# nmoehrle/mvs-texturing

Hardware: AMD Instinct MI355X
Metric: faces/sec through view-selection (data-cost + MRF) (higher is better)
Workload: dtype f32

## Files before the change

include/mvs_viewsel_blocks.h:

```cpp
#ifndef MVS_VIEWSEL_BLOCKS_H
#define MVS_VIEWSEL_BLOCKS_H
#include "mvs_viewsel.h"
#ifdef __cplusplus
extern "C" {
#endif

mvs_status mvs_ctx_dc_get_max(mvs_ctx* ctx, float* dst_device);
mvs_status mvs_ctx_dc_set_max(mvs_ctx* ctx, const float* src_device);
mvs_status mvs_ctx_dc_get_histogram(mvs_ctx* ctx, uint32_t* dst_device);
mvs_status mvs_ctx_dc_set_histogram(mvs_ctx* ctx, const uint32_t* src_device);
mvs_status mvs_ctx_costs_export(mvs_ctx* ctx, uint32_t* counts_device, uint16_t* view_id_device, float* cost_device);

enum { MVS_MRF_MSG = 0, MVS_MRF_LAB = 1, MVS_MRF_GAIN = 2, MVS_MRF_BEST_LAB = 3,
       MVS_MRF_MSG_LAB = 4 };
mvs_status mvs_ctx_mrf_setup(mvs_ctx* ctx, const uint32_t* adj_ptr, const uint32_t* adj, int adj_on_device,
                             const mvs_mrf_params* params);
mvs_status mvs_ctx_mrf_sweep_phase(mvs_ctx* ctx, uint32_t phase, uint32_t node_begin, uint32_t node_end);
mvs_status mvs_ctx_mrf_setup_marked(mvs_ctx* ctx, const uint32_t* adj_ptr, const uint32_t* adj, int adj_on_device,
                                    const mvs_mrf_params* params, const uint8_t* marks_device);
mvs_status mvs_ctx_mrf_sweep_phase_part(mvs_ctx* ctx, uint32_t phase, uint32_t node_begin, uint32_t node_end, int part);
mvs_status mvs_ctx_mrf_sweep(mvs_ctx* ctx, uint32_t node_begin, uint32_t node_end);
mvs_status mvs_ctx_mrf_layout(mvs_ctx* ctx, uint32_t* in_off_host, uint64_t n_edges);
mvs_status mvs_ctx_mrf_gather(mvs_ctx* ctx, int which, const uint32_t* idx_device, uint64_t n, void* dst_device);
mvs_status mvs_ctx_mrf_scatter(mvs_ctx* ctx, int which, const uint32_t* idx_device, uint64_t n, const void* src_device);
mvs_status mvs_ctx_mrf_energy(mvs_ctx* ctx, int which_sel, uint32_t node_begin, uint32_t node_end, uint64_t* dst_device);
mvs_status mvs_ctx_mrf_keep_best(mvs_ctx* ctx);
mvs_status mvs_ctx_mrf_step(mvs_ctx* ctx, const uint64_t* energy_device);
mvs_status mvs_ctx_mrf_poll(mvs_ctx* ctx, uint32_t step, mvs_mrf_progress* out);
mvs_status mvs_ctx_mrf_icm_gain(mvs_ctx* ctx, uint32_t node_begin, uint32_t node_end);
mvs_status mvs_ctx_mrf_icm_apply(mvs_ctx* ctx, uint32_t node_begin, uint32_t node_end, uint32_t* moved_device);
mvs_status mvs_ctx_mrf_labels(mvs_ctx* ctx, uint32_t node_begin, uint32_t node_end, uint32_t* labels_device,
                              uint32_t* unseen_out);

#ifdef __cplusplus
}
#endif
#endif
```

mvs-texturing_amd/csrc/api.hip:

```cpp
#include "ctx.h"

#include <atomic>
#include <cmath>
#include <cstdio>
#include <cstdlib>
#include <cstring>
#include <chrono>
#include <mutex>
#include <string>
#include <thread>
#include <vector>

namespace mvs {
void dc_phase1(mvs_ctx* ctx, const mvs_settings* st);
void dc_phase2(mvs_ctx* ctx);
void dc_phase3(mvs_ctx* ctx, mvs_dc_stats* stats);
void undistort_image(mvs_ctx* ctx, const uint8_t* d_src, uint8_t* d_dst, int w, int h, double flen, double d0, double d1);
void dc_prune_labels(mvs_ctx* ctx, uint32_t kmax);
void dc_postprocess(mvs_ctx* ctx, uint32_t nf, uint32_t n_views, const uint32_t* h_ptr, const uint16_t* h_view_rev, const float* h_q_rev, const float* h_col_rev, const mvs_settings* st);
void mrf_setup(mvs_ctx* ctx, const mvs_mrf_params* params);
void mrf_sweep(mvs_ctx* ctx, uint32_t nb0, uint32_t ne0);
void mrf_energy(mvs_ctx* ctx, bool best, uint32_t nb0, uint32_t ne0, bool reduce = true);
void mrf_keep_best(mvs_ctx* ctx);
void mrf_exact_costs(mvs_ctx* ctx, uint32_t nb0, uint32_t ne0);
// ... 192 lines not shown
            if (!ev[k]) MVS_HIP(hipEventCreateWithFlags(&ev[k], hipEventDisableTiming));
        }
    }
    void release() {
        std::lock_guard<std::mutex> lock(m);
        for (unsigned k = 0; k < SLOTS; ++k) { if (ev[k]) (void)hipEventDestroy(ev[k]); if (buf[k]) (void)hipHostFree(buf[k]); ev[k] = nullptr; buf[k] = nullptr; used[k] = false; }
    }
};
constexpr int RING_DEVICES = 16;
UploadRing g_ring[RING_DEVICES];
unsigned upload_threads() {
    if (const char* e = getenv("MVS_UPLOAD_THREADS")) return (unsigned)std::max(1, std::min(atoi(e), (int)UploadRing::MAX_THREADS));
    return std::max(1u, std::min(UploadRing::MAX_THREADS, std::thread::hardware_concurrency() / 2));
}
void upload_through_ring(mvs_ctx* ctx, const std::vector<UploadPiece>& pieces) {
    if (ctx->device < 0 || ctx->device >= RING_DEVICES) throw StatusError(MVS_ERR_UNSUPPORTED, "upload ring: device index out of range");
    UploadRing& R = g_ring[ctx->device];
    std::lock_guard<std::mutex> lock(R.m);
    struct Chunk { const uint8_t* src; uint8_t* dst; size_t n; };
    std::vector<Chunk> chunks;
    for (const UploadPiece& p : pieces) for (size_t o = 0; o < p.bytes; o += UploadRing::SLOT) chunks.push_back(Chunk{p.src + o, p.dst + o, std::min(UploadRing::SLOT, p.bytes - o)});
    const unsigned T = (unsigned)std::max<size_t>(1, std::min<size_t>(upload_threads(), chunks.size()));
    R.ensure(2 * T);
    hipStream_t s = ctx->stream; const int device = ctx->device;
    struct Drain { hipStream_t s; UploadRing& R; ~Drain() { (void)hipStreamSynchronize(s); for (bool& u : R.used) u = false; } } drain{s, R};
    std::mutex em; std::string error; std::atomic<bool> failed{false};
    auto work = [&](unsigned t) {
        try {
            MVS_HIP(hipSetDevice(device));
            unsigned turn = 0;
            for (size_t c = t; c < chunks.size() && !failed.load(std::memory_order_relaxed); c += T, turn ^= 1u) {
                const unsigned k = 2 * t + turn;
                if (R.used[k]) MVS_HIP(hipEventSynchronize(R.ev[k]));
                memcpy(R.buf[k], chunks[c].src, chunks[c].n);
                MVS_HIP(hipMemcpyAsync(chunks[c].dst, R.buf[k], chunks[c].n, hipMemcpyHostToDevice, s));
                MVS_HIP(hipEventRecord(R.ev[k], s));
                R.used[k] = true;
            }
        } catch (const std::exception& e) { failed.store(true); std::lock_guard<std::mutex> l(em); if (error.empty()) error = e.what(); }
    };
    struct Joiner { std::vector<std::thread> th; ~Joiner() { for (auto& x : th) if (x.joinable()) x.join(); } } pool;
    pool.th.reserve(T);
    std::vector<unsigned> mine{0u};
    for (unsigned t = 1; t < T; ++t) {
        try { pool.th.emplace_back(work, t); } catch (const std::system_error&) { mine.push_back(t); }
    }
    for (unsigned t : mine) work(t);
    for (auto& x : pool.th) x.join();
    if (failed.load()) throw HipError("image upload: " + error);
}
}

extern "C" {

const char* mvs_last_error(void) { return g_last_error.c_str(); }

const char* mvs_status_string(mvs_status s) {
    switch (s) {
        case MVS_OK: return "ok";
        case MVS_ERR_INVALID: return "invalid argument";
        case MVS_ERR_TOO_MANY_FACES: return "Exeeded maximal number of faces";
        case MVS_ERR_TOO_MANY_VIEWS: return "Exeeded maximal number of views";
        case MVS_ERR_LABELING: return "Incorrect labeling";
        case MVS_ERR_HIP: return "HIP error";
        case MVS_ERR_STATE: return "invalid call order";
        case MVS_ERR_UNSUPPORTED: return "unsupported";
    }
    return "?";
}

void mvs_mrf_default_params(mvs_mrf_params* p) {
    p->max_sweeps = 200; p->min_sweeps = 20; p->window = 5; p->min_improvement = 0.005f;
    p->damping = 0.2f; p->rho = 0.8f; p->icm_iters = 50; p->region_rounds = 0;
}
void mvs_default_settings(mvs_settings* s) {
    s->data_term = MVS_DATA_TERM_GMI; s->outlier_removal = MVS_OUTLIER_NONE; s->geometric_visibility_test = 1;
}

mvs_status mvs_ctx_create(int device, mvs_ctx** out) {
    if (!out) return fail(MVS_ERR_INVALID, "out is null");
    *out = nullptr;
    MVS_API_BEGIN
    int n = 0;
    if (hipGetDeviceCount(&n) != hipSuccess || n <= 0) throw HipError("no HIP device available (this library has no CPU fallback)");
    if (device < 0 || device >= n) throw StatusError(MVS_ERR_INVALID, "bad device index");
    MVS_HIP(hipSetDevice(device));
    mvs_ctx* c = new mvs_ctx;
    c->device = device;
    MVS_HIP(hipStreamCreateWithFlags(&c->stream, hipStreamNonBlocking));
    c->own_stream = true;
    c->cos_limit = compute_cos_limit();
    if (const char* e = getenv("MVS_INFO_WAVE_AREA")) c->info_wave_area = std::max(0, atoi(e));
    if (const char* e = getenv("MVS_MRF_WIDE")) c->mrf_wide = atoi(e) != 0;
    if (const char* e = getenv("MVS_BVH_UPPER_MIN_FACES")) c->bvh_upper_min_faces = (uint32_t)std::max(0ll, atoll(e));
    c->counters.ensure(64);
    *out = c;
    MVS_API_END
}

void mvs_ctx_destroy(mvs_ctx* ctx) {
    if (!ctx) return;
    (void)hipSetDevice(ctx->device);
    (void)hipStreamSynchronize(ctx->stream);
    for (auto* b : ctx->own_rgb) delete b;
    if (ctx->sweep_exec) (void)hipGraphExecDestroy(ctx->sweep_exec);
    if (ctx->cap_stream) (void)hipStreamDestroy(ctx->cap_stream);
    if (ctx->aux_stream) { (void)hipStreamSynchronize(ctx->aux_stream); (void)hipStreamDestroy(ctx->aux_stream); }
    if (ctx->ev_fork) (void)hipEventDestroy(ctx->ev_fork);
    if (ctx->ev_join) (void)hipEventDestroy(ctx->ev_join);
    if (ctx->h_kd_flags) (void)hipHostFree(ctx->h_kd_flags);
    if (ctx->h_icm) (void)hipHostFree(ctx->h_icm);
    if (ctx->h_rb) (void)hipHostFree(ctx->h_rb);
    if (ctx->h_seq) (void)hipHostFree(ctx->h_seq);
    if (ctx->h_ring) (void)hipHostFree(ctx->h_ring);
    if (ctx->own_stream && ctx->stream) (void)hipStreamDestroy(ctx->stream);
    delete ctx;
}

mvs_status mvs_ctx_set_stream(mvs_ctx* ctx, void* hip_stream) {
    if (!ctx) return fail(MVS_ERR_INVALID, "ctx is null");
    MVS_API_BEGIN
    MVS_HIP(hipStreamSynchronize(ctx->stream));
    if (ctx->own_stream && ctx->stream) MVS_HIP(hipStreamDestroy(ctx->stream));
    ctx->stream = (hipStream_t)hip_stream; ctx->own_stream = false;
    MVS_API_END
}

mvs_status mvs_ctx_synchronize(mvs_ctx* ctx) {
    if (!ctx) return fail(MVS_ERR_INVALID, "ctx is null");
    MVS_API_BEGIN
    MVS_HIP(hipStreamSynchronize(ctx->stream));
    MVS_API_END
}

mvs_status mvs_set_option(mvs_ctx* ctx, const char* name, int64_t value) {
    if (!ctx || !name) return fail(MVS_ERR_INVALID, "null argument");
    const std::string n(name);
    if (n == "count_rays") ctx->count_rays = value != 0;
    else if (n == "stats") ctx->stats = value != 0;
    else if (n == "verbose") ctx->verbose = value != 0;
    else if (n == "info_wave_area") ctx->info_wave_area = (int)std::max<int64_t>(0, std::min<int64_t>(value, 1 << 30));
    else if (n == "info_wave_area_words") ctx->info_wave_area_words = (int)std::max<int64_t>(1, std::min<int64_t>(value, 1 << 30));
    else if (n == "info_words") ctx->info_words = value != 0;
    else if (n == "info_cert_shift") ctx->info_cert_shift = (int)std::max<int64_t>(0, std::min<int64_t>(value, 40));
    else if (n == "max_labels") { if (value < 0 || value > 65535) return fail(MVS_ERR_INVALID, "max_labels: 0 (off) .. 65535"); ctx->max_labels = (int)value; }
    else if (n == "profile") ctx->profile = value != 0;
    else if (n == "prep_fused") ctx->prep_fused = value != 0;
    else if (n == "ray_xcd") ctx->ray_xcd = (int)value;
    else if (n == "mrf_xcd") ctx->mrf_xcd = (int)value;
    else if (n == "mrf_lag") ctx->mrf_lag = (int)value;
    else if (n == "shard_peer_push") ctx->shard_peer_push = value != 0;
    else if (n == "mrf_force_generic") ctx->mrf_force_generic = value != 0;
    else if (n == "mrf_wide") ctx->mrf_wide = value != 0;
    else if (n == "mrf_graph") ctx->mrf_graph = value != 0;
    else if (n == "mrf_late_old") ctx->mrf_late_old = (int)value;
    else if (n == "mrf_damp_period") ctx->mrf_damp_period = (int)std::max<int64_t>(0, std::min<int64_t>(value, 64));
    else if (n == "mrf_run_pad") ctx->mrf_run_pad = (value == 16) ? 16 : 4;
    else if (n == "mrf_blocks_per_cu") ctx->mrf_blocks_per_cu = std::max(0, (int)value);
    else if (n == "bvh_caller_order") ctx->bvh_caller_order = value != 0;
    else if (n == "dc_overlap_prep") ctx->dc_overlap_prep = value != 0;
    else if (n == "bvh_upper_min_faces") { ctx->kd_disabled = false; ctx->bvh_upper_min_faces = (uint32_t)std::max<int64_t>(0, std::min<int64_t>(value, 0xFFFFFFFFll)); ctx->order_pinned = false; }
    else if (n == "bvh_window") { ctx->kd_disabled = false; ctx->bvh_window = (uint32_t)std::max<int64_t>(0, std::min<int64_t>(value, 0x40000000)); ctx->order_pinned = false; }
    else if (n == "face_order") { ctx->face_order = value != 0 ? 1 : 0; ctx->order_pinned = false; }
    else return fail(MVS_ERR_INVALID, "unknown option " + n);
    return MVS_OK;
}

mvs_status mvs_ctx_get_profile(mvs_ctx* ctx, char* buf, size_t buf_size) {
    if (!ctx || !buf || buf_size < 3) return fail(MVS_ERR_INVALID, "null argument");
    MVS_API_BEGIN
    MVS_HIP(hipStreamSynchronize(ctx->stream));
    std::vector<std::string> names; std::vector<double> ms; std::vector<int> cnt;
    for (auto& sp : ctx->prof_spans) {
        float t = 0.0f;
        MVS_HIP(hipEventElapsedTime(&t, sp.a, sp.b));
        size_t k = 0;
        for (; k < names.size(); ++k) if (names[k] == sp.name) break;
        if (k == names.size()) { names.push_back(sp.name); ms.push_back(0.0); cnt.push_back(0); }
        ms[k] += t; cnt[k] += 1;
        if (sp.owns_a) ctx->prof_pool.push_back(sp.a);
        ctx->prof_pool.push_back(sp.b);
    }
    ctx->prof_spans.clear();
    std::string out = "{";
    for (size_t k = 0; k < names.size(); ++k) {
        char tmp[160];
        snprintf(tmp, sizeof(tmp), "%s\"%s\": [%.6f, %d]", k ? ", " : "", names[k].c_str(), ms[k], cnt[k]);
        out += tmp;
    }
    out += "}";
    if (out.size() + 1 > buf_size) throw StatusError(MVS_ERR_INVALID, "profile buffer too small");
    memcpy(buf, out.c_str(), out.size() + 1);
    MVS_API_END
}

mvs_status mvs_scene_set_mesh(mvs_ctx* ctx, const mvs_mesh* mesh, int on_device) {
    if (!ctx || !mesh || !mesh->verts || !mesh->faces || !mesh->face_normals) return fail(MVS_ERR_INVALID, "null argument");
    MVS_API_BEGIN
    MVS_HIP(hipSetDevice(ctx->device));
    const size_t NV = mesh->n_verts, F = mesh->n_faces;
    if (on_device) {
        ctx->d_verts = mesh->verts; ctx->d_faces = mesh->faces; ctx->d_normals = mesh->face_normals;
    } else {
        ctx->own_verts.ensure(3 * NV + 4); ctx->own_faces.ensure(3 * F + 4); ctx->own_normals.ensure(3 * F + 4);
        MVS_HIP(hipMemcpyAsync(ctx->own_verts.p, mesh->verts, 3 * NV * sizeof(float), hipMemcpyHostToDevice, ctx->stream));
        MVS_HIP(hipMemcpyAsync(ctx->own_faces.p, mesh->faces, 3 * F * sizeof(uint32_t), hipMemcpyHostToDevice, ctx->stream));
        MVS_HIP(hipMemcpyAsync(ctx->own_normals.p, mesh->face_normals, 3 * F * sizeof(float), hipMemcpyHostToDevice, ctx->stream));
        MVS_HIP(hipStreamSynchronize(ctx->stream));
        ctx->d_verts = ctx->own_verts.p; ctx->d_faces = ctx->own_faces.p; ctx->d_normals = ctx->own_normals.p;
    }
    ctx->n_verts = mesh->n_verts; ctx->n_faces = mesh->n_faces;
    ctx->face_begin = 0; ctx->face_end = mesh->n_faces;
    ctx->have_costs = false; ctx->dc_phase = 0;
    ctx->order_pinned = false; ctx->iv = nullptr; ctx->kd_disabled = false; ctx->kd_pending = 0;
    MVS_API_END
}

static mvs_status set_views_impl(mvs_ctx* ctx, const mvs_view* views, uint32_t n_views, int rgb_on_device, const mvs_image_source* src);
mvs_status mvs_scene_set_views(mvs_ctx* ctx, const mvs_view* views, uint32_t n_views, int rgb_on_device) { return set_views_impl(ctx, views, n_views, rgb_on_device, nullptr); }
mvs_status mvs_scene_set_views_from(mvs_ctx* ctx, const mvs_view* views, uint32_t n_views, const mvs_image_source* src) {
    if (!src || !src->acquire || !src->release) return fail(MVS_ERR_INVALID, "null argument");
    return set_views_impl(ctx, views, n_views, 0, src);
}
static mvs_status set_views_impl(mvs_ctx* ctx, const mvs_view* views, uint32_t n_views, int rgb_on_device, const mvs_image_source* src) {
    if (!ctx || (!views && n_views)) return fail(MVS_ERR_INVALID, "null argument");
    MVS_API_BEGIN
    MVS_HIP(hipSetDevice(ctx->device));
    if (rgb_on_device) { for (auto* b : ctx->own_rgb) delete b; ctx->own_rgb.clear(); }
    else { while (ctx->own_rgb.size() > n_views) { delete ctx->own_rgb.back(); ctx->own_rgb.pop_back(); } }
    ctx->h_views.assign(n_views, ViewParams{});
    struct Pinned {
        hipStream_t s; std::vector<void*> ptrs;
        ~Pinned() { if (ptrs.empty()) return; (void)hipStreamSynchronize(s); for (void* p : ptrs) (void)hipHostUnregister(p); }
    } pinned{ctx->stream, {}};
    UploadRoute route = rgb_on_device ? UploadRoute::Pageable : upload_route();
    if (src && route == UploadRoute::Register) route = UploadRoute::Ring;
    std::vector<UploadPiece> pieces;
    struct Held {
        const mvs_image_source* src; std::vector<uint32_t> views;
        void release_all() { for (uint32_t j : views) src->release(src->user, j); views.clear(); }
        ~Held() { if (src) release_all(); }
    } held{src, {}};
    const uint32_t in_flight = src ? std::max<uint32_t>(1u, src->max_in_flight ? src->max_in_flight : 4u) : 0u;
    auto flush_batch = [&]() {
        if (!pieces.empty()) upload_through_ring(ctx, pieces);
        pieces.clear();
        MVS_HIP(hipStreamSynchronize(ctx->stream));
        held.release_all();
    };
    for (uint32_t j = 0; j < n_views; ++j) {
        mvs_view v = views[j];
        if (src) {
            if (v.width < 2 || v.height < 2) throw StatusError(MVS_ERR_INVALID, "view " + std::to_string(j) + ": bad image");
            v.rgb = src->acquire(src->user, j);
            if (!v.rgb) throw StatusError(MVS_ERR_INVALID, "view " + std::to_string(j) + ": the image source has no image");
            held.views.push_back(j);
        }
        if (v.width < 2 || v.height < 2 || !v.rgb) throw StatusError(MVS_ERR_INVALID, "view " + std::to_string(j) + ": bad image");
        ViewParams& p = ctx->h_views[j];
        memcpy(p.pos, v.pos, sizeof(p.pos)); memcpy(p.viewdir, v.viewdir, sizeof(p.viewdir));
        memcpy(p.K, v.K, sizeof(p.K)); memcpy(p.w2c, v.w2c, sizeof(p.w2c));
        p.width = v.width; p.height = v.height;
        if (rgb_on_device) p.rgb = v.rgb;
        else {
            if (ctx->own_rgb.size() <= j) ctx->own_rgb.push_back(new DBuf<uint8_t>());
            auto* b = ctx->own_rgb[j];
            const size_t bytes = (size_t)v.width * v.height * 3;
            b->ensure(bytes + 16);
            p.rgb = b->p;
            if (route == UploadRoute::Ring && bytes >= (1u << 18)) { pieces.push_back(UploadPiece{v.rgb, b->p, bytes}); if (src && held.views.size() >= in_flight) flush_batch(); continue; }
            if (route == UploadRoute::Register && bytes >= (1u << 20) && hipHostRegister(const_cast<uint8_t*>(v.rgb), bytes, hipHostRegisterDefault) == hipSuccess) pinned.ptrs.push_back(const_cast<uint8_t*>(v.rgb));
            else (void)hipGetLastError();
            MVS_HIP(hipMemcpyAsync(b->p, v.rgb, bytes, hipMemcpyHostToDevice, ctx->stream));
            if (src && held.views.size() >= in_flight) flush_batch();
        }
    }
    if (src) flush_batch();
    if (!pieces.empty()) upload_through_ring(ctx, pieces);
    MVS_HIP(hipStreamSynchronize(ctx->stream));
    ctx->n_views = n_views;
    ctx->have_costs = false; ctx->dc_phase = 0;
    MVS_API_END
}

mvs_status mvs_scene_set_face_range(mvs_ctx* ctx, uint32_t begin, uint32_t end) {
    if (!ctx) return fail(MVS_ERR_INVALID, "ctx is null");
    if (begin > end || end > ctx->n_faces) return fail(MVS_ERR_INVALID, "bad face range");
    ctx->face_begin = begin; ctx->face_end = end;
    ctx->have_costs = false; ctx->dc_phase = 0;
    return MVS_OK;
}

mvs_status mvs_ctx_dc_phase1(mvs_ctx* ctx, const mvs_settings* settings) {
    if (!ctx || !settings) return fail(MVS_ERR_INVALID, "null argument");
    MVS_API_BEGIN
    MVS_HIP(hipSetDevice(ctx->device));
    dc_phase1(ctx, settings);
    MVS_API_END
}
mvs_status mvs_ctx_dc_phase2(mvs_ctx* ctx) {
    if (!ctx) return fail(MVS_ERR_INVALID, "ctx is null");
    MVS_API_BEGIN
    MVS_HIP(hipSetDevice(ctx->device));
    dc_phase2(ctx);
    MVS_API_END
}
// ... 515 lines not shown
```

mvs-texturing_amd/csrc/ctx.h:

```cpp
#pragma once
#include <hip/hip_runtime.h>
#include <stdint.h>
#include <string.h>
#include <algorithm>
#include <stdexcept>
#include <string>
#include <vector>

#include "../../include/mvs_viewsel.h"
#include "dmath.h"

namespace mvs {

struct HipError : std::runtime_error {
    explicit HipError(const std::string& m) : std::runtime_error(m) {}
};
struct StatusError : std::runtime_error {
    mvs_status st;
    StatusError(mvs_status s, const std::string& m) : std::runtime_error(m), st(s) {}
};

#define MVS_HIP(expr)                                                                          \
    do {                                                                                       \
        hipError_t _e = (expr);                                                                \
// ... 39 lines not shown
    HBuf() = default;
    HBuf(const HBuf&) = delete;
    HBuf& operator=(const HBuf&) = delete;
};

struct alignas(128) Node4 {
    float b[4][6];
    uint32_t nchild;
    uint32_t pad_[7];
    __host__ __device__ float lo(int a, int c) const { return b[c][a]; }
    __host__ __device__ float hi(int a, int c) const { return b[c][3 + a]; }
};
static_assert(sizeof(Node4) == 128, "Node4 must be one 128-byte line");

struct BvhDev {
    const Node4* nodes;
    const float4* tris;
    uint32_t level_off[16];
    uint32_t level_cnt[16];
    int32_t top;
    uint32_t n_leaves;
};

struct ProfSpan { std::string name; hipEvent_t a, b; bool owns_a; };

struct MrfEdge {
    uint32_t in_off;
    uint32_t out_off;
    uint32_t kj;
};

struct alignas(16) NodeDesc {
    uint32_t rec;
    uint32_t id;
    uint32_t in_off[3];
    uint32_t out_off[3];
    uint32_t kk;
    uint32_t nbr[3];
};
static_assert(sizeof(NodeDesc) == 48, "NodeDesc must be 48 bytes");

}

struct mvs_ctx {
    int device = 0;
    hipStream_t stream = nullptr;
    bool own_stream = false;
    bool verbose = false;
    bool profile = false;
    std::vector<mvs::ProfSpan> prof_spans; std::vector<hipEvent_t> prof_pool;
    bool prep_fused = true;
    bool stats = false;
    bool count_rays = false;
    bool dc_overlap_prep = true;
    uint32_t* h_kd_flags = nullptr; int kd_pending = 0; bool kd_disabled = false;
    uint32_t* h_rb = nullptr; uint32_t* d_rb = nullptr; uint32_t rb_seq = 0;
    hipStream_t aux_stream = nullptr; hipEvent_t ev_fork = nullptr, ev_join = nullptr;
    uint32_t bvh_upper_min_faces = 1000000;
    uint32_t bvh_window = 262144;
    mvs::DBuf<float> kd_c[2][3]; mvs::DBuf<uint32_t> kd_id[2], kd_hist, kd_cursor, kd_tie, kd_pivot, kd_box;
    bool bvh_caller_order = false;
    int ray_xcd = 1;
    int info_wave_area = 32;
    int info_wave_area_words = 384;
    bool info_words = true;
    int info_cert_shift = 0;
    uint32_t dc_stats_deferred = 0;
    int max_labels = 0;
    float cos_limit = 0.0f;

    uint32_t n_verts = 0, n_faces = 0, n_views = 0;
    uint32_t face_begin = 0, face_end = 0;
    const float* d_verts = nullptr; const uint32_t* d_faces = nullptr; const float* d_normals = nullptr;
    mvs::DBuf<float> own_verts, own_normals; mvs::DBuf<uint32_t> own_faces;
    std::vector<mvs::ViewParams> h_views;
    mvs::DBuf<mvs::ViewParams> d_views;
    std::vector<mvs::DBuf<uint8_t>*> own_rgb;
    mvs::DBuf<uint8_t> gmi_all;
    mvs::DBuf<uint8_t> lum_all;
    mvs::DBuf<uint32_t> mask_all;
    mvs::DBuf<uint32_t> mask_zero, mask_tmp;
    mvs::DBuf<uint32_t> msum_all;
    std::vector<size_t> gmi_off, mask_off, msum_off;
    mvs::DBuf<size_t> view_off;
    bool mesh_dirty = true, views_dirty = true;

    int face_order = 1;
    mvs::DBuf<float> i_verts, i_normals; mvs::DBuf<uint32_t> i_faces, f_perm, f_pos, f_tmp;
    const float* iv = nullptr; const uint32_t* ifc = nullptr; const float* inr = nullptr;
    bool mesh_ordered = false;
    bool order_pinned = false;
    const uint32_t* t_perm = nullptr; const uint32_t* t_pos = nullptr;
    mvs::DBuf<uint32_t> u_ptr, u_cnt; mvs::DBuf<uint16_t> u_view; mvs::DBuf<float> u_cost, u_q;
    bool u_valid = false, u_q_valid = false;
    mvs::DBuf<unsigned long long> fp_acc;
    mvs::HBuf<uint32_t> stage_ptr; mvs::HBuf<uint16_t> stage_view[2]; mvs::HBuf<float> stage_cost[2];

    mvs::DBuf<mvs::Node4> bvh_nodes; mvs::DBuf<float4> bvh_tris;
    mvs::DBuf<uint32_t> sort_k, sort_k2, sort_v, sort_v2; mvs::DBuf<char> sort_tmp;
    mvs::DBuf<float> lvl_box_a, lvl_box_b; mvs::DBuf<float> scene_box;
    mvs::BvhDev bvh{};
    mvs::DBuf<uint32_t> vf_ptr, vf_cursor, vf;
    mvs::DBuf<uint32_t> vperm, vpos;
    const uint32_t* tri_order = nullptr;

    mvs::DBuf<unsigned long long> pass_bits, need_bits, occl_bits, surv_bits;
    mvs::DBuf<uint32_t> pass_base;
    mvs::DBuf<uint32_t> pass_face;
    mvs::DBuf<unsigned long long> defer_bits; mvs::DBuf<uint32_t> defer_base; mvs::DBuf<uint2> defer_list; mvs::DBuf<uint32_t> rewalk_list;
    mvs::DBuf<float> pq;
    mvs::DBuf<float> pcol;
    mvs::DBuf<uint32_t> face_cnt, scan_tmp;
    mvs::DBuf<unsigned long long> counters;
    mvs::DBuf<float> max_q; mvs::DBuf<uint32_t> hist; mvs::DBuf<float> pctl;
    mvs::DBuf<uint32_t> pre_ptr; mvs::DBuf<uint16_t> pre_view; mvs::DBuf<float> pre_q; mvs::DBuf<float> pre_col;
    mvs::DBuf<uint8_t> pre_inl;
    mvs::DBuf<uint32_t> csr_ptr; mvs::DBuf<uint16_t> csr_view; mvs::DBuf<float> csr_cost; mvs::DBuf<float> csr_q;
    uint32_t csr_faces = 0, csr_views = 0; uint64_t csr_nnz = 0;
    const uint32_t* r_ptr = nullptr; const uint16_t* r_view = nullptr; const float* r_cost = nullptr;
    bool csr_q_valid = false;
    bool have_costs = false;
    mvs_settings dc_settings{}; mvs_dc_stats dc_stats{}; int dc_phase = 0;

    mvs::DBuf<unsigned long long> g_keys, g_keys2; mvs::DBuf<uint32_t> g_vals, g_vals2, g_pos, g_cnt, g_adj_ptr, g_adj, g_faces; mvs::DBuf<float> g_normals;
    uint64_t g_adj_entries = 0; bool have_adj = false;

    mvs::DBuf<uint32_t> p_label_ptr, p_comp_ptr, p_comp_faces, p_parent, p_root, p_state, p_flag, p_pos, p_roots, p_roots2, p_rlab, p_rlab2, p_adj_ptr, p_adj, p_labels;

    mvs::DBuf<uint32_t> rg_parent, rg_root, rg_size, rg_bestl, rg_lose, rg_flag, rg_pos, rg_cstart, rg_have, rg_cfirst, rg_name;
    mvs::DBuf<unsigned long long> rg_gain, rg_cur, rg_key, rg_key2, rg_ck, rg_sum; mvs::DBuf<long long> rg_cgain; mvs::DBuf<uint2> rg_cut;

    mvs::DBuf<uint32_t> m_adj_ptr, m_adj, a_stage_ptr, a_stage; const uint32_t* r_adj_ptr = nullptr; const uint32_t* r_adj = nullptr;
    uint32_t r_adj_edges = 0; bool r_adj_edges_known = false;
    mvs::DBuf<mvs::NodeDesc> m_desc; mvs::DBuf<uint8_t> m_ident; mvs::DBuf<uint32_t> m_rec; uint64_t m_rec_words = 0; bool m_fast = false; int mrf_blocks_per_cu = 0 , mrf_xcd = 1, mrf_late_old = 1, mrf_run_pad = 4;
    mvs::DBuf<mvs::MrfEdge> m_edge; mvs::DBuf<uint32_t> m_size, m_rev ; mvs::DBuf<uint16_t> m_map;
    mvs::DBuf<uint8_t> m_msg_a;
    mvs::DBuf<uint32_t> m_sel, m_sel2, m_cand; mvs::DBuf<float> m_gain;
    mvs::DBuf<uint32_t> m_lab; mvs::DBuf<float> m_cost;
    uint32_t m_stride = 0;
    bool exact_valid = false; uint32_t exact_nb = 0, exact_ne = 0;
    uint32_t* b_sel = nullptr; uint32_t* b_lab = nullptr; float* b_cost = nullptr; bool best_resolved = false;
    mvs::DBuf<unsigned long long> m_energy; mvs::DBuf<uint32_t> m_moved; mvs::DBuf<uint32_t> m_alist; bool icm_dirty_valid = false;
    uint32_t m_n_adj = 0;
    uint32_t m_energy_blocks = 0;
    bool m_energy_from_sweep = false;
    uint64_t m_total = 0; uint32_t m_kmax = 0, m_degmax = 0;
    mvs::DBuf<uint32_t> m_colour, m_perm, m_tmp_a, m_tmp_b, m_tmp_c, m_sub; mvs::DBuf<uint8_t> m_cls; uint32_t m_colours = 0, m_n_fast = 0; std::vector<uint32_t> m_sub_begin;
    const uint32_t* m_colour_in = nullptr;
    const uint8_t* m_bnd = nullptr;
    int mrf_damp_period = 4;
    int mrf_force_generic = 0;
    int mrf_wide = 1;
    bool m_wide_layout = false;
    uint32_t m_range_nb = 0, m_range_ne = 0; std::vector<uint32_t> m_range_q;
    uint32_t m_sweep_no = 0;
    mvs_mrf_params m_params{};
    static constexpr uint32_t RING = 16;
    static constexpr uint32_t ICM_RING = 8;
    uint32_t* h_icm = nullptr; uint32_t* d_icm = nullptr; uint32_t icm_seq = 0;
    mvs::DBuf<mvs_mrf_progress> m_state; mvs::DBuf<unsigned long long> m_hist; mvs::DBuf<uint32_t> m_ctl;
    int mrf_graph = 1; hipStream_t cap_stream = nullptr; hipGraphExec_t sweep_exec = nullptr; uint32_t graph_launches = 0, graph_updates = 0, graph_instantiations = 0;
    mvs_mrf_progress* h_ring = nullptr; mvs_mrf_progress* d_ring = nullptr ; uint32_t steps_issued = 0; int mrf_lag = 1;
    int shard_peer_push = 1;
    uint32_t* h_seq = nullptr; uint32_t* d_seq = nullptr; uint32_t seq_base = 0;
};

namespace mvs {
struct Prof {
    mvs_ctx* c; size_t idx; bool on;
    Prof(mvs_ctx* ctx, const char* name) : c(ctx), idx(0), on(ctx->profile) {
        if (!on) return;
        auto get = [&]() { hipEvent_t e; if (!c->prof_pool.empty()) { e = c->prof_pool.back(); c->prof_pool.pop_back(); } else { MVS_HIP(hipEventCreate(&e)); } return e; };
        ProfSpan sp{name, get(), get(), true};
        MVS_HIP(hipEventRecord(sp.a, c->stream));
        idx = c->prof_spans.size(); c->prof_spans.push_back(sp);
    }
    void end() { if (on) { MVS_HIP(hipEventRecord(c->prof_spans[idx].b, c->stream)); on = false; } }
    ~Prof() { if (on) (void)hipEventRecord(c->prof_spans[idx].b, c->stream); }
};
struct ProfChain {
    mvs_ctx* c; hipEvent_t prev; bool on;
    static hipEvent_t get(mvs_ctx* c) { hipEvent_t e; if (!c->prof_pool.empty()) { e = c->prof_pool.back(); c->prof_pool.pop_back(); } else { MVS_HIP(hipEventCreate(&e)); } return e; }
    explicit ProfChain(mvs_ctx* ctx) : c(ctx), prev(nullptr), on(ctx->profile) {}
    void begin() { if (on && !prev) { prev = get(c); MVS_HIP(hipEventRecord(prev, c->stream)); first = true; } }
    void mark(const char* name) {
        if (!on) return;
        begin();
        hipEvent_t e = get(c);
        MVS_HIP(hipEventRecord(e, c->stream));
        c->prof_spans.push_back(ProfSpan{name, prev, e, first});
        first = false; prev = e;
    }
    bool first = false;
};
struct RoctxRange { explicit RoctxRange(const char* name); ~RoctxRange(); bool on; };
int default_device();
enum { MRF_PART_ALL = 0, MRF_PART_BOUNDARY = 1, MRF_PART_INTERIOR = 2 };
void ensure_report_ring(mvs_ctx* ctx);
void report_u32(mvs_ctx* ctx, const uint32_t* d_src, uint32_t* d_dst, uint32_t seq_slot, uint32_t seq);
void wait_report(mvs_ctx* ctx, uint32_t seq_slot, uint32_t seq);
void read_words(mvs_ctx* ctx, const void* d_src, void* out, uint32_t n_words);
void read_block(mvs_ctx* ctx, const void* d_src, void* out, size_t bytes);
void exclusive_scan_u32(mvs_ctx* ctx, const uint32_t* in, uint32_t* out, size_t n, uint32_t* d_total);
uint64_t sum_u32(mvs_ctx* ctx, const uint32_t* in, size_t n);
}
```

mvs-texturing_amd/csrc/k_mrf.hip:

```cpp
#include "ctx.h"
#include <rocprim/rocprim.hpp>
#include <atomic>

namespace mvs {

namespace {

constexpr uint16_t MAP_NONE = 0xFFFF;
constexpr uint32_t MSG_BASE = MVS_MRF_MSG_BASE;

typedef uint8_t msg_t;
struct MsgQ { float scale, step; };
__device__ __forceinline__ MsgQ msg_q(float lam) { return MsgQ{255.0f / lam, lam / 255.0f}; }
template <class T> __device__ __forceinline__ T ld_off(const void* base, uint32_t byte_off) { return *reinterpret_cast<const T*>(reinterpret_cast<const char*>(base) + byte_off); }
template <class T> __device__ __forceinline__ void st_off(void* base, uint32_t byte_off, T v) { *reinterpret_cast<T*>(reinterpret_cast<char*>(base) + byte_off) = v; }
__device__ __forceinline__ float min_raw(float a, float b) { float r; asm("v_min_f32 %0, %1, %2" : "=v"(r) : "v"(a), "v"(b)); return r; }
template <bool DAMP>
__device__ __forceinline__ uint32_t msg_pack_s(float raw_s, float alpha, float old_code, uint32_t byte, uint32_t word) {
    return __builtin_amdgcn_cvt_pk_u8_f32(DAMP ? __builtin_fmaf(old_code, alpha, raw_s) : raw_s, byte, word);
}
template <bool DAMP>
__device__ __forceinline__ uint32_t msg_pack(float raw, float oms, float alpha, float old_code, uint32_t byte, uint32_t word) {
    const float v = DAMP ? __builtin_fmaf(old_code, alpha, raw * oms) : raw * oms;
    return __builtin_amdgcn_cvt_pk_u8_f32(v, byte, word);
// ... 167 lines not shown
        for (int t = 0; t < 4; ++t) { oj[t] = orig ? orig[j[t]] : j[t]; cj[t] = __hip_atomic_load(colour + j[t], __ATOMIC_RELAXED, __HIP_MEMORY_SCOPE_AGENT); }
#pragma unroll
        for (int t = 0; t < 4; ++t) {
            if (j[t] == i || !mrf_key_less(oj[t], oi)) continue;
            if (cj[t] == NO_COLOUR) ready = false; else used |= 1ull << cj[t];
        }
    }
    if (ready) {
        if (used == ~0ull) { pending[1] = 1u; used = 0ull; }
        __hip_atomic_store(colour + i, (uint32_t)__builtin_ctzll(~used), __ATOMIC_RELAXED, __HIP_MEMORY_SCOPE_AGENT);
    } else *pending = 1u;
}
constexpr uint32_t N_SUB = 320;
constexpr uint32_t SUB_GENERIC = 256;
constexpr uint32_t N_KEY = 2 * N_SUB;
__global__ void mrf_sortkey_kernel(const uint32_t* __restrict__ colour, const uint8_t* __restrict__ cls, const uint8_t* __restrict__ bnd, uint32_t F, uint32_t* __restrict__ key) {
    const uint32_t i = blockIdx.x * blockDim.x + threadIdx.x;
    if (i < F) { const uint32_t c = colour[i], k = cls[i]; key[i] = 2u * ((k == CLS_GENERIC) ? SUB_GENERIC + c : 4u * c + k) + ((bnd && bnd[i]) ? 0u : 1u); }
}
__global__ void mrf_sub_begin_kernel(const uint32_t* __restrict__ sorted, uint32_t F, uint32_t* __restrict__ sub_begin) {
    const uint32_t c = blockIdx.x * blockDim.x + threadIdx.x;
    if (c > N_KEY) return;
    uint32_t lo = 0, hi = F;
    while (lo < hi) { const uint32_t mid = (lo + hi) >> 1; if (sorted[mid] < c) lo = mid + 1; else hi = mid; }
    sub_begin[c] = lo;
}
__global__ void mrf_sub_range_kernel(const uint32_t* __restrict__ perm, const uint32_t* __restrict__ sub_begin,
                                     uint32_t nb, uint32_t ne, uint32_t* __restrict__ out) {
    const uint32_t c = blockIdx.x * blockDim.x + threadIdx.x;
    if (c >= N_KEY) return;
    const uint32_t cb = sub_begin[c], ce = sub_begin[c + 1];
    uint32_t lo = cb, hi = ce;
    while (lo < hi) { const uint32_t mid = (lo + hi) >> 1; if (perm[mid] < nb) lo = mid + 1; else hi = mid; }
    out[2 * c] = lo;
    hi = ce;
    while (lo < hi) { const uint32_t mid = (lo + hi) >> 1; if (perm[mid] < ne) lo = mid + 1; else hi = mid; }
    out[2 * c + 1] = lo;
}
constexpr int MAX_LAYOUT_COLOURS = 8;
__global__ void mrf_nodesize_kernel(const uint32_t* __restrict__ perm, const uint32_t* __restrict__ colour, const uint32_t* __restrict__ adj_ptr,
                                    const uint32_t* __restrict__ adj, const uint32_t* __restrict__ size, const uint32_t* __restrict__ rev, uint32_t F, uint32_t n_col,
                                    uint32_t* __restrict__ nsz) {
    const uint32_t q = blockIdx.x * blockDim.x + threadIdx.x;
    if (q > F) return;
    uint32_t acc[MAX_LAYOUT_COLOURS];
#pragma unroll
    for (int b = 0; b < MAX_LAYOUT_COLOURS; ++b) acc[b] = 0;
    if (q < F) {
        const uint32_t j = perm[q];
        const uint32_t ra = adj_ptr[j], rz = adj_ptr[j + 1];
        for (uint32_t rb = ra; rb < rz; rb += 4) {
            uint32_t i[4], e[4], b[4], sz[4];
#pragma unroll
            for (int t = 0; t < 4; ++t) { const bool on = rb + t < rz; i[t] = on ? adj[rb + t] : j; e[t] = on ? rev[rb + t] : 0xFFFFFFFFu; }
#pragma unroll
            for (int t = 0; t < 4; ++t) { b[t] = (n_col > 1) ? colour[i[t]] : 0u; sz[t] = (e[t] != 0xFFFFFFFFu) ? size[e[t]] : 0u; }
#pragma unroll
            for (int t = 0; t < 4; ++t)
#pragma unroll
                for (int c = 0; c < MAX_LAYOUT_COLOURS; ++c) acc[c] += ((uint32_t)c == b[t]) ? sz[t] : 0u;
        }
    }
#pragma unroll
    for (int b = 0; b < MAX_LAYOUT_COLOURS; ++b) if ((uint32_t)b < n_col) nsz[(size_t)b * (F + 1) + q] = acc[b];
}
__global__ void mrf_inoff_kernel(const uint32_t* __restrict__ perm, const uint32_t* __restrict__ colour, const uint32_t* __restrict__ adj_ptr,
                                 const uint32_t* __restrict__ adj, const uint32_t* __restrict__ size, const uint32_t* __restrict__ rev, const uint32_t* __restrict__ noff,
                                 uint32_t F, uint32_t n_col, uint32_t* __restrict__ in_off) {
    const uint32_t q = blockIdx.x * blockDim.x + threadIdx.x;
    if (q >= F) return;
    const uint32_t j = perm[q];
    uint32_t off[MAX_LAYOUT_COLOURS];
#pragma unroll
    for (int b = 0; b < MAX_LAYOUT_COLOURS; ++b) off[b] = ((uint32_t)b < n_col) ? noff[(size_t)b * (F + 1) + q] : 0u;
    const uint32_t ra = adj_ptr[j], rz = adj_ptr[j + 1];
    for (uint32_t rb = ra; rb < rz; rb += 4) {
        uint32_t i[4], e[4], b[4], sz[4];
#pragma unroll
        for (int t = 0; t < 4; ++t) { const bool on = rb + t < rz; i[t] = on ? adj[rb + t] : j; e[t] = on ? rev[rb + t] : 0xFFFFFFFFu; }
#pragma unroll
        for (int t = 0; t < 4; ++t) { b[t] = (n_col > 1) ? colour[i[t]] : 0u; sz[t] = (e[t] != 0xFFFFFFFFu) ? size[e[t]] : 0u; }
#pragma unroll
        for (int t = 0; t < 4; ++t) {
            if (e[t] == 0xFFFFFFFFu) continue;
            uint32_t o = 0;
#pragma unroll
            for (int c = 0; c < MAX_LAYOUT_COLOURS; ++c) { if ((uint32_t)c == b[t]) { o = off[c]; off[c] += sz[t]; } }
            in_off[e[t]] = o;
        }
    }
}

__global__ void mrf_edge_kernel(const uint32_t* __restrict__ col_ptr, const uint32_t* __restrict__ adj_ptr, const uint32_t* __restrict__ adj,
                                uint32_t F, const uint32_t* __restrict__ in_off, const uint32_t* __restrict__ size, const uint32_t* __restrict__ rev, MrfEdge* __restrict__ edge) {
    const uint32_t i = blockIdx.x * blockDim.x + threadIdx.x;
    if (i >= F) return;
    const uint32_t e0 = adj_ptr[i], e1 = adj_ptr[i + 1];
    for (uint32_t eb = e0; eb < e1; eb += 4) {
        uint32_t j[4], r[4], io[4], sz[4], oo[4], kj[4];
#pragma unroll
        for (int t = 0; t < 4; ++t) { const bool on = eb + t < e1; j[t] = on ? adj[eb + t] : i; r[t] = on ? rev[eb + t] : 0xFFFFFFFFu; io[t] = on ? in_off[eb + t] : 0u; sz[t] = on ? size[eb + t] : 0u; }
#pragma unroll
        for (int t = 0; t < 4; ++t) { oo[t] = (r[t] != 0xFFFFFFFFu) ? in_off[r[t]] : 0u; kj[t] = col_ptr[j[t] + 1] - col_ptr[j[t]]; }
#pragma unroll
        for (int t = 0; t < 4; ++t) {
            if (eb + t >= e1) continue;
            const bool has = r[t] != 0xFFFFFFFFu;
            MrfEdge m;
            m.in_off = MSG_BASE + io[t];
            m.out_off = has ? MSG_BASE + oo[t] : 0u;
            m.kj = (sz[t] > 0 && has) ? kj[t] : 0u;
            edge[eb + t] = m;
        }
    }
}

constexpr uint32_t MAP_TILE = 256;
__global__ void __launch_bounds__(256) mrf_map_kernel(const uint32_t* __restrict__ col_ptr, const uint16_t* __restrict__ view_id, const uint32_t* __restrict__ adj_ptr,
                               const uint32_t* __restrict__ adj, uint32_t F, const MrfEdge* __restrict__ edge, const uint8_t* __restrict__ cls, uint16_t* __restrict__ map) {
    __shared__ uint16_t s_l[16][MAP_TILE];
    const uint32_t i = (blockIdx.x * blockDim.x + threadIdx.x) >> 4;
    const uint32_t gl = threadIdx.x & 15;
    if (i >= F) return;
    uint16_t* tile = s_l[threadIdx.x >> 4];
    const uint32_t p0 = col_ptr[i], K = col_ptr[i + 1] - p0;
    for (uint32_t e = adj_ptr[i]; e < adj_ptr[i + 1]; ++e) {
        const MrfEdge m = edge[e];
        if (m.kj == 0 || cls[adj[e]] != CLS_GENERIC) continue;
        const uint32_t q0 = col_ptr[adj[e]];
        const bool in_lds = m.kj <= MAP_TILE;
        if (in_lds) for (uint32_t t = gl; t < m.kj; t += 16) tile[t] = view_id[q0 + t];
        for (uint32_t t = gl; t < K; t += 16) {
            const uint16_t key = view_id[p0 + t];
            uint32_t lo = 0, hi = m.kj;
            if (in_lds) { while (lo < hi) { const uint32_t mid = (lo + hi) >> 1; if (tile[mid] < key) lo = mid + 1; else hi = mid; } }
            else { while (lo < hi) { const uint32_t mid = (lo + hi) >> 1; if (view_id[q0 + mid] < key) lo = mid + 1; else hi = mid; } }
            const uint16_t found = (lo < m.kj) ? (in_lds ? tile[lo] : view_id[q0 + lo]) : (uint16_t)0;
            map[m.in_off + t] = (lo < m.kj && found == key) ? (uint16_t)lo : MAP_NONE;
        }
    }
}

constexpr uint32_t REC_BASE = 256;
constexpr float COST_SCALE = 65535.0f;
__device__ __forceinline__ uint32_t cost_code(float c) { return (uint32_t)(c * COST_SCALE + 0.5f); }
__device__ __forceinline__ float cost_value(uint32_t code) { return (float)code * (1.0f / 65535.0f); }
__device__ __forceinline__ uint32_t label_position(const uint16_t* __restrict__ view_id, uint32_t p0, uint32_t K, uint32_t l) {
    uint32_t lo = 0, hi = K;
    const uint32_t key = l - 1u;
    while (lo < hi) { const uint32_t mid = (lo + hi) >> 1; if ((uint32_t)view_id[p0 + mid] < key) lo = mid + 1; else hi = mid; }
    return lo < K ? lo : K - 1u;
}

__global__ void __launch_bounds__(256) mrf_ident_kernel(const uint32_t* __restrict__ col_ptr, const uint16_t* __restrict__ view_id, const uint32_t* __restrict__ adj_ptr,
                                                        const uint32_t* __restrict__ adj, uint32_t F, const MrfEdge* __restrict__ edge, const uint8_t* __restrict__ cls,
                                                        uint8_t* __restrict__ ident) {
    const uint32_t i = (blockIdx.x * blockDim.x + threadIdx.x) >> 4;
    const uint32_t gl = threadIdx.x & 15;
    if (i >= F || cls[i] == CLS_GENERIC) return;
    const uint32_t p0 = col_ptr[i], K = col_ptr[i + 1] - p0;
    const uint32_t e0 = adj_ptr[i], e1 = adj_ptr[i + 1];
    for (uint32_t e = e0; e < e1; e += 3) {
        uint32_t kj[3], q0[3];
#pragma unroll
        for (int k = 0; k < 3; ++k) {
            const bool on = e + k < e1;
            kj[k] = on ? edge[e + k].kj : 0u;
            q0[k] = col_ptr[on ? adj[e + k] : i];
        }
        uint32_t same = 0;
#pragma unroll
        for (int k = 0; k < 3; ++k) same |= (kj[k] != 0u && kj[k] == K) ? (1u << k) : 0u;
        if (same) {
            for (uint32_t t = gl; t < K; t += 16) {
                const uint32_t v = view_id[p0 + t];
#pragma unroll
                for (int k = 0; k < 3; ++k)
                    if ((same >> k) & 1u) { if (view_id[q0[k] + t] != v) same &= ~(1u << k); }
            }
            for (int o = 8; o > 0; o >>= 1) same &= __shfl_xor(same, o, 16);
        }
        if (gl < 3 && e + gl < e1 && kj[gl] != 0u) ident[e + gl] = (uint8_t)((same >> gl) & 1u);
    }
}
__global__ void mrf_recsize_kernel(const uint32_t* __restrict__ col_ptr, const uint32_t* __restrict__ adj_ptr, const MrfEdge* __restrict__ edge,
                                   const uint8_t* __restrict__ ident, const uint8_t* __restrict__ cls, const uint32_t* __restrict__ perm, uint32_t F, uint32_t wide,
                                   uint32_t* __restrict__ rsz, uint32_t* __restrict__ qpos) {
    const uint32_t q = blockIdx.x * blockDim.x + threadIdx.x;
    if (q > F) return;
    uint32_t w = 0;
    if (q < F) {
        const uint32_t i = perm[q], K = col_ptr[i + 1] - col_ptr[i];
        qpos[i] = q;
        if (K && cls[i] != CLS_GENERIC) {
            w = (K + 3u) & ~3u;
            const bool w8 = wide != 0u && cls[i] == 1u;
            const uint32_t e0 = adj_ptr[i], e1 = adj_ptr[i + 1];
            for (uint32_t eb = e0; eb < e1; eb += 4) {
                uint32_t kj[4], id[4];
#pragma unroll
                for (int t = 0; t < 4; ++t) { const bool on = eb + t < e1; kj[t] = on ? edge[eb + t].kj : 0u; id[t] = on ? ident[eb + t] : 1u; }
#pragma unroll
                for (int t = 0; t < 4; ++t) if (kj[t] && !id[t]) w += w8 ? 2u * ((kj[t] + 7u) >> 3) : (kj[t] + 3u) >> 2;
            }
            w = (w + 3u) & ~3u;
        }
    }
    rsz[q] = w;
}
__global__ void __launch_bounds__(256) mrf_record_kernel(const uint32_t* __restrict__ col_ptr, const uint16_t* __restrict__ view_id, const float* __restrict__ cost,
                                                         const uint32_t* __restrict__ adj_ptr, const uint32_t* __restrict__ adj, const MrfEdge* __restrict__ edge,
                                                         const uint8_t* __restrict__ ident, const uint8_t* __restrict__ cls, const uint32_t* __restrict__ qpos, const uint32_t* __restrict__ roff,
                                                         uint32_t F, uint32_t wide, uint32_t* __restrict__ rec) {
    __shared__ uint16_t s_l[16][256];
    const uint32_t i = (blockIdx.x * blockDim.x + threadIdx.x) >> 4;
    const uint32_t gl = threadIdx.x & 15;
    if (i >= F) return;
    const uint32_t p0 = col_ptr[i], K = col_ptr[i + 1] - p0;
    const uint32_t ci = cls[i];
    if (K == 0 || ci == CLS_GENERIC) return;
    const bool w8 = wide != 0u && ci == 1u;
    const uint32_t rs = w8 ? 8u : 8u << ci, none_byte = w8 ? 64u : (ci < 3u ? 4u * rs : 0xFFu);
    const uint32_t lmask = w8 ? 7u : 3u, lshift = w8 ? 3u : 2u;
    const uint32_t q = qpos[i];
    uint16_t* tile = s_l[threadIdx.x >> 4];
    uint32_t* out = rec + REC_BASE + roff[q];
    const uint32_t K4 = (K + 3u) & ~3u;
    const uint32_t e0 = adj_ptr[i], deg = adj_ptr[i + 1] - e0;
    uint32_t kj3[3], q03[3];
    {
        uint32_t kj[3], idn[3], nb[3];
#pragma unroll
        for (uint32_t d = 0; d < 3; ++d) { const bool on = d < deg; kj[d] = on ? edge[e0 + d].kj : 0u; idn[d] = on ? (uint32_t)ident[e0 + d] : 1u; nb[d] = on ? adj[e0 + d] : i; }
#pragma unroll
        for (uint32_t d = 0; d < 3; ++d) { kj3[d] = (kj[d] != 0u && idn[d] == 0u) ? kj[d] : 0u; q03[d] = col_ptr[nb[d]]; }
    }
    for (uint32_t t = gl; t < K4; t += 16) {
        uint32_t w = 0u;
        if (t < K) { const uint32_t v = view_id[p0 + t]; tile[t] = (uint16_t)v; w = (cost_code(cost[p0 + t]) << 16) | v; }
        out[t] = w;
    }
    uint32_t pos = K4;
#pragma unroll
    for (uint32_t d = 0; d < 3; ++d) {
        const uint32_t kj = kj3[d];
        if (kj == 0) continue;
        const uint32_t q0 = q03[d], nw = w8 ? 2u * ((kj + 7u) >> 3) : (kj + 3u) >> 2;
        for (uint32_t wI = gl; wI < nw; wI += 16) {
            uint32_t key[4], lo[4] = {0u, 0u, 0u, 0u};
#pragma unroll
            for (uint32_t r = 0; r < 4; ++r) { const uint32_t t2 = 4u * wI + r; key[r] = (t2 < kj) ? (uint32_t)view_id[q0 + t2] : 0xFFFFFFFFu; }
            for (uint32_t n = K; n > 1u;) {
                const uint32_t half = n >> 1;
#pragma unroll
                for (uint32_t r = 0; r < 4; ++r) lo[r] += ((uint32_t)tile[lo[r] + half - 1u] < key[r]) ? half : 0u;
                n -= half;
            }
            uint32_t word = 0u;
#pragma unroll
            for (uint32_t r = 0; r < 4; ++r) {
                uint32_t at = lo[r] + (((uint32_t)tile[lo[r]] < key[r]) ? 1u : 0u);
                const uint32_t byte = (at < K && (uint32_t)tile[at < K ? at : 0u] == key[r]) ? (at & lmask) * rs + (at >> lshift) : none_byte;
                word |= byte << (8 * r);
            }
            out[pos + wI] = word;
        }
        pos += nw;
    }
    for (uint32_t t = pos + gl; t < ((pos + 3u) & ~3u); t += 16) out[t] = 0u;
}
__global__ void mrf_desc_kernel(const uint32_t* __restrict__ col_ptr, const uint32_t* __restrict__ adj_ptr, const uint32_t* __restrict__ adj,
                                const MrfEdge* __restrict__ edge, const uint8_t* __restrict__ ident, const uint32_t* __restrict__ perm,
                                const uint32_t* __restrict__ colour, const uint32_t* __restrict__ roff, uint32_t n_fast, NodeDesc* __restrict__ desc) {
    const uint32_t q = blockIdx.x * blockDim.x + threadIdx.x;
    if (q >= n_fast) return;
    const uint32_t i = perm[q];
    NodeDesc nd;
    const uint32_t k = col_ptr[i + 1] - col_ptr[i];
    nd.rec = k ? REC_BASE + roff[q] : 0u; nd.id = i; nd.kk = k;
    const uint32_t e0 = adj_ptr[i], deg = adj_ptr[i + 1] - e0, ci = colour[i];
    for (int d = 0; d < 3; ++d) {
        MrfEdge m; m.in_off = 0; m.out_off = 0; m.kj = 0;
        uint32_t flag_ident = 0, flag_low = 0, nb = i;
        if ((uint32_t)d < deg) { nb = adj[e0 + d]; flag_low = (colour[nb] < ci) ? 1u : 0u; }
        if ((uint32_t)d < deg && k > 0) {
            m = edge[e0 + d];
            if (m.kj && ident[e0 + d]) flag_ident = 1u;
            if (m.kj == 0) { m.in_off = 0; m.out_off = 0; }
        }
        nd.in_off[d] = m.in_off | flag_low; nd.out_off[d] = m.out_off | flag_ident; nd.kk |= m.kj << (8 + 8 * d); nd.nbr[d] = nb;
    }
    desc[q] = nd;
}

template <int G, bool DAMP, bool XCD, bool LATE_OLD>
__global__ void __launch_bounds__(256) mrf_sweep4_kernel(const NodeDesc* __restrict__ desc, const uint32_t* __restrict__ rec, msg_t* msg,
                                                         const mvs_mrf_progress* __restrict__ st, uint32_t* lab2, uint32_t buf_stride,
                                                         uint32_t node_begin , uint32_t node_end, float rho, float alpha,
                                                         unsigned long long* __restrict__ partial) {
    const msg_t* mo = msg; msg_t* mn = msg;
    constexpr int NPB = 256 / G;
    constexpr int TS = G == 8 ? 40 : G == 16 ? 80 : 4 * G + 4;
    __shared__ float s_c[NPB * TS];
    __shared__ unsigned long long s_e[8];
    const int grp = threadIdx.x / G, gl = threadIdx.x % G;
    float* __restrict__ tile = s_c + grp * TS;
    if (st->stopped) return;
    if (gl == 0) tile[4 * G] = INFINITY;
    __syncthreads();
    const uint32_t wofs = st->w * buf_stride;
    uint32_t* lab = lab2 + wofs;
    const float lam = 1.0f / rho;
    const MsgQ mq = msg_q(lam);
    const float kappa = rho * mq.step, nstep = -mq.step, oms = (1.0f - alpha) * mq.scale, lam_s = lam * oms;
    constexpr float HUGE_COST = 1e30f;
    const uint32_t stride = gridDim.x * NPB;
    uint32_t vb = blockIdx.x;
    if (XCD && (gridDim.x & 7u) == 0u) vb = (blockIdx.x & 7u) * (gridDim.x >> 3) + (blockIdx.x >> 3);
    uint32_t i = node_begin + vb * NPB + grp;
    const uint32_t last = node_end - 1;
    const uint32_t n_iter = (node_end - node_begin + stride - 1) / stride;
    const uint32_t t0 = 4u * gl;
    const uint32_t ident_word = 0x03020100u * (uint32_t)G + 0x01010101u * (uint32_t)gl;
    struct Raw { uint4 lw; uint32_t in[3], map[3], nl[3], old[3]; };
    const uint32_t t0b = 4u * t0, glb = 4u * (uint32_t)gl;
    auto issue = [&](const NodeDesc& d, Raw& r) {
        const uint32_t K = d.kk & 0xFFu, recb = 4u * d.rec;
        r.lw = ld_off<uint4>(rec, recb + t0b);
        uint32_t mposb = recb + 4u * ((K + 3u) & ~3u) + glb;
#pragma unroll
        for (int e = 0; e < 3; ++e) {
            r.in[e] = ld_off<uint32_t>(mo, (d.in_off[e] & ~3u) + t0);
            r.map[e] = ld_off<uint32_t>(rec, mposb);
            if (!(d.out_off[e] & 1u)) mposb += (((d.kk >> (8 + 8 * e)) & 0xFFu) + 3u) & ~3u;
            r.nl[e] = ld_off<uint32_t>(lab, 4u * d.nbr[e]);
            if (DAMP) r.old[e] = ld_off<uint32_t>(mo, (d.out_off[e] & ~3u) + t0); else r.old[e] = d.out_off[e];
        }
    };
    NodeDesc cur = ld_off<NodeDesc>(desc, (uint32_t)sizeof(NodeDesc) * min(i, last));
    Raw rw; issue(cur, rw);
    NodeDesc nxt = ld_off<NodeDesc>(desc, (uint32_t)sizeof(NodeDesc) * min(i + stride, last));
    uint32_t acc_e = 0u, acc_c = 0u;
#pragma unroll 2
    for (uint32_t it = 0; it < n_iter; ++it, i += stride) {
        const bool node_ok = i < node_end;
        Raw rn; issue(nxt, rn);
        const NodeDesc nn = ld_off<NodeDesc>(desc, (uint32_t)sizeof(NodeDesc) * min(i + 2u * stride, last));
        const uint32_t K = node_ok ? (cur.kk & 0xFFu) : 0u;
        bool ok[4];
#pragma unroll
        for (int r = 0; r < 4; ++r) ok[r] = t0 + r < K;
        uint32_t kj3[3], o_out[3]; bool ident[3], low[3];
#pragma unroll
        for (int d = 0; d < 3; ++d) {
            kj3[d] = node_ok ? ((cur.kk >> (8 + 8 * d)) & 0xFFu) : 0u;
            ident[d] = (cur.out_off[d] & 1u) != 0u; low[d] = (cur.in_off[d] & 1u) != 0u && kj3[d] != 0u;
            o_out[d] = cur.out_off[d] & ~3u;
        }
        const uint32_t lw[4] = {rw.lw.x, rw.lw.y, rw.lw.z, rw.lw.w};
        const uint32_t* r_in = rw.in; const uint32_t* r_map = rw.map; const uint32_t* nl = rw.nl; const uint32_t* r_old = rw.old;
        float cf[3][4], b[4];
#pragma unroll
        for (int r = 0; r < 4; ++r) {
#pragma unroll
            for (int d = 0; d < 3; ++d) cf[d][r] = (float)((r_in[d] >> (8 * r)) & 0xFFu);
            const float D = ok[r] ? cost_value(lw[r] >> 16) : HUGE_COST;
            b[r] = __builtin_fmaf(kappa, (cf[0][r] + cf[1][r]) + cf[2][r], D);
        }
        float cv[3][4];
#pragma unroll
        for (int d = 0; d < 3; ++d)
#pragma unroll
            for (int r = 0; r < 4; ++r) cv[d][r] = __builtin_fmaf(nstep, cf[d][r], b[r]) * oms;
        float gm = fminf(fminf(b[0], b[1]), fminf(b[2], b[3]));
        float cm0 = fminf(fminf(cv[0][0], cv[0][1]), fminf(cv[0][2], cv[0][3])), cm1 = fminf(fminf(cv[1][0], cv[1][1]), fminf(cv[1][2], cv[1][3])),
              cm2 = fminf(fminf(cv[2][0], cv[2][1]), fminf(cv[2][2], cv[2][3]));
        group_min_fused4<G>(gm, cm0, cm1, cm2);
        const float cmin3[3] = {cm0, cm1, cm2};
        uint32_t bt = (b[3] == gm) ? t0 + 3u : 0xFFFFFFFFu;
        bt = (b[2] == gm) ? t0 + 2u : bt; bt = (b[1] == gm) ? t0 + 1u : bt; bt = (b[0] == gm) ? t0 : bt;
        bt = group_min_fused<G>(bt);
#pragma unroll
        for (int d = 0; d < 3; ++d) {
#pragma unroll
            for (int r = 0; r < 4; ++r) tile[r * G + gl] = cv[d][r] - cmin3[d];
            const uint32_t mw = ident[d] ? ident_word : r_map[d];
            uint32_t w = 0u;
#pragma unroll
            for (int r = 0; r < 4; ++r) {
                const uint32_t mp = (mw >> (8 * r)) & 0xFFu;
                const uint32_t slot = (G < 64) ? mp : ((mp == 0xFFu) ? (uint32_t)(4 * G) : mp);
                w = msg_pack_s<DAMP>(min_raw(tile[slot], lam_s), alpha, (float)((r_old[d] >> (8 * r)) & 0xFFu), (uint32_t)r, w);
            }
            if (t0 < kj3[d]) st_off<uint32_t>(mn, o_out[d] + t0, w);
        }
        const bool owner = node_ok && ((K > 0u) ? ((bt >> 2) == (uint32_t)gl) : (gl == 0));
        if (owner) {
            const uint32_t r = bt & 3u;
            const uint32_t wsel = (r == 0u) ? lw[0] : (r == 1u) ? lw[1] : (r == 2u) ? lw[2] : lw[3];
            const uint32_t my_lab = (K > 0u) ? (wsel & 0xFFFFu) + 1u : 0u;
            const uint32_t my_code = (K > 0u) ? (wsel >> 16) : 65535u;
            const uint32_t idb = 4u * cur.id;
            st_off<uint32_t>(lab, idb, my_lab);
            acc_e += my_code;
// ... 329 lines not shown
__global__ void __launch_bounds__(256) mrf_icm_apply_kernel(const uint32_t* __restrict__ col_ptr, const uint16_t* __restrict__ view_id, const float* __restrict__ cost,
                                                            const uint32_t* __restrict__ adj_ptr, const uint32_t* __restrict__ adj,
                                                            const float* __restrict__ gain, const uint32_t* __restrict__ cand,
                                                            uint32_t* sel, uint32_t* lab, float* selcost,
                                                            uint32_t node_begin, uint32_t node_end, uint32_t* __restrict__ moved ,
                                                            uint32_t* __restrict__ alist ,
                                                            const uint32_t* __restrict__ orig ) {
    const uint32_t i = node_begin + blockIdx.x * blockDim.x + threadIdx.x;
    bool mv = false;
    if (i < node_end) {
        const float gi = gain[i];
        if (gi > 0.0f) {
            bool win = true;
            for (uint32_t e = adj_ptr[i]; e < adj_ptr[i + 1] && win; ++e) {
                const uint32_t j = adj[e];
                if (lab[j] == 0u) continue;
                const float gj = gain[j];
                if (gj > gi || (gj == gi && (orig ? orig[j] < orig[i] : j < i))) win = false;
            }
            if (win) mv = true;
        }
    }
    if (mv) {
        const uint32_t p0 = col_ptr[i], t = cand[i];
        sel[i] = t; lab[i] = (uint32_t)view_id[p0 + t] + 1u; selcost[i] = cost[p0 + t];
        if (alist) {
            const uint32_t e0 = adj_ptr[i], e1 = adj_ptr[i + 1];
            uint32_t w = atomicAdd(&moved[1], 1u + (e1 - e0));
            alist[w++] = i;
            for (uint32_t e = e0; e < e1; ++e) alist[w++] = adj[e];
        }
    }
    const unsigned long long b = __ballot(mv);
    if ((threadIdx.x & 63) == 0 && b) atomicAdd(moved, (uint32_t)__popcll(b));
}

__global__ void mrf_argmin_unary_kernel(const uint32_t* __restrict__ col_ptr, const uint16_t* __restrict__ view_id, const float* __restrict__ cost, uint32_t F,
                                        uint32_t* __restrict__ sel, uint32_t* __restrict__ lab, float* __restrict__ selcost) {
    const uint32_t i = blockIdx.x * blockDim.x + threadIdx.x;
    if (i >= F) return;
    const uint32_t p0 = col_ptr[i], K = col_ptr[i + 1] - p0;
    uint32_t bt = 0;
    for (uint32_t t = 1; t < K; ++t) if (cost[p0 + t] < cost[p0 + bt]) bt = t;
    sel[i] = bt;
    lab[i] = K ? (uint32_t)view_id[p0 + bt] + 1u : 0u;
    selcost[i] = K ? cost[p0 + bt] : 1.0f;
}

__global__ void mrf_labels_kernel(const uint32_t* __restrict__ lab, uint32_t node_begin, uint32_t node_end, uint32_t n_views,
                                  uint32_t* __restrict__ labels, uint32_t* __restrict__ bad_unseen ,
                                  const uint32_t* __restrict__ orig ,
                                  const uint32_t* __restrict__ foreign ) {
    const uint32_t i = node_begin + blockIdx.x * blockDim.x + threadIdx.x;
    if (i >= node_end) return;
    if (foreign && i == node_begin && *foreign) atomicAdd(&bad_unseen[0], *foreign);
    const uint32_t label = lab[i];
    if (label > n_views) atomicAdd(&bad_unseen[0], 1u);
    if (label == 0u) atomicAdd(&bad_unseen[1], 1u);
    labels[orig ? orig[i] : i - node_begin] = label;
}


__global__ void __launch_bounds__(1024) mrf_step_kernel(mvs_mrf_progress* __restrict__ st, unsigned long long* __restrict__ hist,
                                const unsigned long long* __restrict__ energy, const unsigned long long* __restrict__ partial, uint32_t n_partial,
                                unsigned long long* __restrict__ energy_out, mvs_mrf_progress* __restrict__ ring, uint32_t* __restrict__ ring_seq, uint32_t ring_slots,
                                uint32_t* __restrict__ ctl, int max_sweeps, int min_sweeps, int window, float min_improvement,
                                const unsigned long long* const* __restrict__ peer_tab = nullptr, uint32_t n_peer = 0, uint32_t peer_off = 0) {
    __shared__ unsigned long long su[16], sc[16];
    unsigned long long e_sum = 0, c_sum = 0;
    if (partial) {
        const ulonglong2* pp = reinterpret_cast<const ulonglong2*>(partial);
#pragma unroll 8
        for (uint32_t b = threadIdx.x; b < n_partial; b += 1024u) { const ulonglong2 v = pp[b]; e_sum += v.x; c_sum += v.y; }
        for (int o = 32; o > 0; o >>= 1) { e_sum += __shfl_xor(e_sum, o, 64); c_sum += __shfl_xor(c_sum, o, 64); }
        if ((threadIdx.x & 63) == 0) { su[threadIdx.x >> 6] = e_sum; sc[threadIdx.x >> 6] = c_sum; }
        __syncthreads();
    }
    if (threadIdx.x != 0 || blockIdx.x != 0) return;
    if (partial) {
        e_sum = 0; c_sum = 0;
        for (int k = 0; k < 16; ++k) { e_sum += su[k]; c_sum += sc[k]; }
        energy_out[0] = e_sum; energy_out[1] = c_sum;
    } else if (peer_tab) {
        e_sum = 0; c_sum = 0;
        for (uint32_t q = 0; q < n_peer; ++q) { e_sum += peer_tab[q][peer_off]; c_sum += peer_tab[q][peer_off + 1u]; }
        energy_out[0] = e_sum; energy_out[1] = c_sum;
    }
    mvs_mrf_progress p = *st;
    if (p.stopped) { p.improved = 0u; }
    else {
        const uint32_t sw = p.sweep + 1u;
        const unsigned long long e0 = (partial || peer_tab) ? e_sum : energy[0];
        const bool imp = e0 < p.best;
        if (imp) { p.best = e0; p.best_w = p.w; p.w ^= 1u; }
        p.sweep = sw; p.improved = imp ? 1u : 0u; p.energy = e0;
        hist[sw] = p.best;
        bool stop = false;
        if ((int)sw >= min_sweeps && (int)sw > window) {
            const unsigned long long prev = hist[sw - (uint32_t)window];
            stop = (double)(prev - p.best) < (double)min_improvement * (double)prev;
        }
        if ((int)sw >= max_sweeps) stop = true;
        if (stop) { p.stopped = 1u; p.stop_sweep = sw; }
    }
    *st = p;
    const uint32_t n = ctl[0] + 1u; ctl[0] = n;
    if (ring) {
        const uint32_t slot = n % ring_slots;
        ring[slot] = p;
        __threadfence_system();
        __hip_atomic_store(ring_seq + slot, ctl[1] + n, __ATOMIC_RELEASE, __HIP_MEMORY_SCOPE_SYSTEM);
    }
}
__global__ void report_u32_kernel(const uint32_t* __restrict__ src, uint32_t* __restrict__ dst, uint32_t* __restrict__ dst_seq, uint32_t seq) {
    *dst = *src;
    __threadfence_system();
    __hip_atomic_store(dst_seq, seq, __ATOMIC_RELEASE, __HIP_MEMORY_SCOPE_SYSTEM);
}
__global__ void report_words_kernel(const uint32_t* __restrict__ src, uint32_t n, uint32_t* __restrict__ dst, uint32_t* __restrict__ dst_seq, uint32_t seq) {
    if (threadIdx.x < n) dst[threadIdx.x] = src[threadIdx.x];
    __threadfence_system();
    __syncthreads();
    if (threadIdx.x == 0) __hip_atomic_store(dst_seq, seq, __ATOMIC_RELEASE, __HIP_MEMORY_SCOPE_SYSTEM);
}
__global__ void mrf_flip_kernel(mvs_mrf_progress* __restrict__ st) { st->best_w = st->w; st->w ^= 1u; }

}

constexpr uint32_t EPART_BLOCKS = 2048;

void mrf_setup(mvs_ctx* ctx, const mvs_mrf_params* params) {
    hipStream_t s = ctx->stream;
    const uint32_t F = ctx->csr_faces;
    ctx->m_params = *params;
    if (!(params->rho > 0.0f && params->rho <= 1.0f) || !(params->damping >= 0.0f && params->damping < 1.0f))
        throw StatusError(MVS_ERR_INVALID, "mrf params: need 0 < rho <= 1, 0 <= damping < 1");
    if (params->window < 1 || params->min_sweeps < 0 || !(params->min_improvement >= 0.0f) || params->icm_iters < 0)
        throw StatusError(MVS_ERR_INVALID, "mrf params: need window >= 1, min_sweeps >= 0, min_improvement >= 0, icm_iters >= 0");
    uint32_t E = ctx->r_adj_edges;
    if (!ctx->r_adj_edges_known) {
        MVS_HIP(hipMemcpyAsync(&E, ctx->r_adj_ptr + F, sizeof(uint32_t), hipMemcpyDeviceToHost, s));
        MVS_HIP(hipStreamSynchronize(s));
    }
    ctx->m_size.ensure((size_t)E + 2); ctx->m_edge.ensure((size_t)E + 1); ctx->m_moved.ensure(8 + 2 * 64);
    ctx->m_n_adj = E;
    uint32_t* maxes = ctx->m_moved.p + 4;
    MVS_HIP(hipMemsetAsync(ctx->m_moved.p, 0, 8 * sizeof(uint32_t), s));
    MVS_HIP(hipMemsetAsync(ctx->m_size.p, 0, ((size_t)E + 2) * sizeof(uint32_t), s));
    const unsigned nb = (F + 255) / 256;
    const uint32_t force_generic = (ctx->csr_nnz < 4 || E == 0 || ctx->mrf_force_generic) ? 1u : 0u;
    ctx->m_cls.ensure((size_t)F + 4);
    ctx->m_rev.ensure((size_t)E + 2);
    if (F) { hipLaunchKernelGGL(mrf_size_kernel, dim3(nb), dim3(256), 0, s, ctx->r_ptr, ctx->r_adj_ptr, ctx->r_adj, F, (uint32_t)(ctx->mrf_run_pad == 16 ? 15 : (ctx->mrf_wide ? 7 : 3)), force_generic, ctx->m_size.p, ctx->m_cls.p, maxes, ctx->m_rev.p); MVS_LAUNCH_CHECK(); }
    ctx->m_colour.ensure((size_t)F + 2); ctx->m_perm.ensure((size_t)F + 2); ctx->m_tmp_a.ensure((size_t)MAX_LAYOUT_COLOURS * ((size_t)F + 1) + 72); ctx->m_tmp_b.ensure((size_t)MAX_LAYOUT_COLOURS * ((size_t)F + 1) + 2); ctx->m_tmp_c.ensure((size_t)F + 2);
    ctx->m_colours = 0; ctx->m_sub_begin.assign(N_KEY + 1, 0); ctx->m_n_fast = 0; ctx->m_range_q.clear(); ctx->m_range_nb = ctx->m_range_ne = 0;
    ctx->m_sweep_no = 0;
    if (F) {
        uint32_t* pending = ctx->m_moved.p + 1;
        hipLaunchKernelGGL(mrf_colour_init_kernel, dim3(nb), dim3(256), 0, s, ctx->m_colour.p, ctx->m_tmp_a.p , F); MVS_LAUNCH_CHECK();
        if (ctx->m_colour_in) MVS_HIP(hipMemcpyAsync(ctx->m_colour.p, ctx->m_colour_in, (size_t)F * sizeof(uint32_t), hipMemcpyDeviceToDevice, s));
        for (int round = 0; !ctx->m_colour_in; ++round) {
            if (round >= 4096) throw StatusError(MVS_ERR_HIP, "graph colouring did not terminate");
            MVS_HIP(hipMemsetAsync(pending, 0, sizeof(uint32_t), s));
            for (int k = 0; k < (round == 0 ? 16 : 4); ++k) { hipLaunchKernelGGL(mrf_colour_round_kernel, dim3(nb), dim3(256), 0, s, ctx->r_adj_ptr, ctx->r_adj, ctx->t_perm, F, ctx->m_colour.p, pending); MVS_LAUNCH_CHECK(); }
            uint32_t hp[2] = {0, 0};
            read_words(ctx, pending, hp, 2);
            if (hp[1]) throw StatusError(MVS_ERR_UNSUPPORTED, "adjacency graph needs more than 64 colours (a node with >= 64 mutually constrained neighbours)");
            if (!hp[0]) break;
        }
        MVS_HIP(hipMemsetAsync(ctx->m_moved.p, 0, 4 * sizeof(uint32_t), s));
        hipLaunchKernelGGL(mrf_sortkey_kernel, dim3(nb), dim3(256), 0, s, ctx->m_colour.p, ctx->m_cls.p, ctx->m_bnd, F, ctx->m_tmp_c.p); MVS_LAUNCH_CHECK();
        size_t tmp_bytes = 0;
        MVS_HIP(rocprim::radix_sort_pairs(nullptr, tmp_bytes, ctx->m_tmp_c.p, ctx->m_tmp_b.p, ctx->m_tmp_a.p, ctx->m_perm.p, F, 0, 10, s));
        ctx->sort_tmp.ensure(tmp_bytes + 16);
        MVS_HIP(rocprim::radix_sort_pairs(ctx->sort_tmp.p, tmp_bytes, ctx->m_tmp_c.p, ctx->m_tmp_b.p, ctx->m_tmp_a.p, ctx->m_perm.p, F, 0, 10, s));
        ctx->m_sub.ensure(3 * (size_t)N_KEY + 8);
        hipLaunchKernelGGL(mrf_sub_begin_kernel, dim3((N_KEY + 256) / 256), dim3(256), 0, s, ctx->m_tmp_b.p, F, ctx->m_sub.p); MVS_LAUNCH_CHECK();
        read_block(ctx, ctx->m_sub.p, ctx->m_sub_begin.data(), (N_KEY + 1) * sizeof(uint32_t));
        const std::vector<uint32_t>& sb = ctx->m_sub_begin;
        uint32_t C = 0;
        for (uint32_t c = 0; c < 64; ++c) if (sb[2 * (4 * c + 4)] > sb[2 * (4 * c)] || sb[2 * (SUB_GENERIC + c + 1)] > sb[2 * (SUB_GENERIC + c)]) C = c + 1;
        ctx->m_colours = C;
        ctx->m_n_fast = sb[2 * SUB_GENERIC];
    }
    DBuf<uint32_t>& in_off = ctx->m_sel2;
    in_off.ensure(std::max<size_t>((size_t)E + 2, (size_t)F + 2));
    MVS_HIP(hipMemsetAsync(in_off.p, 0, ((size_t)E + 2) * sizeof(uint32_t), s));
    uint32_t h[3] = {0, 0, 0};
    if (F) {
        if ((uint64_t)E * 4ull + 4ull * (uint64_t)ctx->csr_nnz >= 0xFFFFFFF0ull) {
            const uint64_t total = sum_u32(ctx, ctx->m_size.p, (size_t)E + 1);
            if ((uint64_t)MSG_BASE + total >= 0xFFFFFFF0ull) throw StatusError(MVS_ERR_UNSUPPORTED, "message array exceeds 2^32 elements (shard the graph: DESIGN.md multi-GPU)");
        }
        const uint32_t n_col = (ctx->m_colours >= 2 && ctx->m_colours <= (uint32_t)MAX_LAYOUT_COLOURS) ? ctx->m_colours : 1u;
        const size_t n_ent = (size_t)n_col * ((size_t)F + 1);
        ctx->m_tmp_a.ensure(n_ent + 72); ctx->m_tmp_b.ensure(n_ent + 2);
        hipLaunchKernelGGL(mrf_nodesize_kernel, dim3((F + 256) / 256), dim3(256), 0, s, ctx->m_perm.p, ctx->m_colour.p, ctx->r_adj_ptr, ctx->r_adj, ctx->m_size.p, ctx->m_rev.p, F, n_col, ctx->m_tmp_a.p); MVS_LAUNCH_CHECK();
        exclusive_scan_u32(ctx, ctx->m_tmp_a.p, ctx->m_tmp_b.p, n_ent, nullptr);
        hipLaunchKernelGGL(mrf_inoff_kernel, dim3(nb), dim3(256), 0, s, ctx->m_perm.p, ctx->m_colour.p, ctx->r_adj_ptr, ctx->r_adj, ctx->m_size.p, ctx->m_rev.p, ctx->m_tmp_b.p, F, n_col, in_off.p); MVS_LAUNCH_CHECK();
        MVS_HIP(hipMemcpyAsync(maxes + 2, ctx->m_tmp_b.p + (n_ent - 1), sizeof(uint32_t), hipMemcpyDeviceToDevice, s));
    } else MVS_HIP(hipMemsetAsync(maxes + 2, 0, sizeof(uint32_t), s));
    { uint32_t hm[3]; read_words(ctx, maxes, hm, 3); h[1] = hm[0]; h[2] = hm[1]; h[0] = hm[2]; }
    ctx->m_total = (uint64_t)MSG_BASE + h[0]; ctx->m_kmax = h[1]; ctx->m_degmax = h[2];
    if (ctx->m_total >= 0xFFFFFFF0ull) throw StatusError(MVS_ERR_UNSUPPORTED, "message array exceeds 2^32 elements");
    if (F) { hipLaunchKernelGGL(mrf_edge_kernel, dim3(nb), dim3(256), 0, s, ctx->r_ptr, ctx->r_adj_ptr, ctx->r_adj, F, in_off.p, ctx->m_size.p, ctx->m_rev.p, ctx->m_edge.p); MVS_LAUNCH_CHECK(); }
    ctx->m_ident.ensure((size_t)E + 1);
    MVS_HIP(hipMemsetAsync(ctx->m_ident.p, 0, (size_t)E + 1, s));
    ctx->m_fast = true;
    ctx->m_wide_layout = ctx->mrf_wide != 0;
    const uint32_t n_fast = ctx->m_n_fast, n_generic = F - n_fast;
    if (n_fast) {
        const size_t rec_cap = (size_t)REC_BASE + ctx->csr_nnz + 8 * (size_t)F + ctx->m_total / 4 + (ctx->mrf_wide ? (size_t)ctx->m_n_adj : 0) + 1024;
        ctx->m_rec.ensure(rec_cap);
        MVS_HIP(hipMemsetAsync(ctx->m_rec.p, 0, REC_BASE * sizeof(uint32_t), s));
        hipLaunchKernelGGL(mrf_ident_kernel, dim3((unsigned)(((size_t)F * 16 + 255) / 256)), dim3(256), 0, s, ctx->r_ptr, ctx->r_view, ctx->r_adj_ptr, ctx->r_adj, F, ctx->m_edge.p, ctx->m_cls.p, ctx->m_ident.p); MVS_LAUNCH_CHECK();
        uint32_t* rsz = ctx->m_tmp_a.p; uint32_t* roff = ctx->m_tmp_b.p;
        hipLaunchKernelGGL(mrf_recsize_kernel, dim3((F + 256) / 256), dim3(256), 0, s, ctx->r_ptr, ctx->r_adj_ptr, ctx->m_edge.p, ctx->m_ident.p, ctx->m_cls.p, ctx->m_perm.p, F, (uint32_t)(ctx->mrf_wide ? 1 : 0), rsz, ctx->m_tmp_c.p); MVS_LAUNCH_CHECK();
        exclusive_scan_u32(ctx, rsz, roff, (size_t)F + 1, nullptr);
        hipLaunchKernelGGL(mrf_record_kernel, dim3((unsigned)(((size_t)F * 16 + 255) / 256)), dim3(256), 0, s, ctx->r_ptr, ctx->r_view, ctx->r_cost, ctx->r_adj_ptr, ctx->r_adj,
                           ctx->m_edge.p, ctx->m_ident.p, ctx->m_cls.p, ctx->m_tmp_c.p , roff, F, (uint32_t)(ctx->mrf_wide ? 1 : 0), ctx->m_rec.p); MVS_LAUNCH_CHECK();
        ctx->m_desc.ensure((size_t)F + 1);
        hipLaunchKernelGGL(mrf_desc_kernel, dim3((n_fast + 255) / 256), dim3(256), 0, s, ctx->r_ptr, ctx->r_adj_ptr, ctx->r_adj, ctx->m_edge.p, ctx->m_ident.p, ctx->m_perm.p, ctx->m_colour.p, roff, n_fast, ctx->m_desc.p); MVS_LAUNCH_CHECK();
    }
    if (n_generic) {
        ctx->m_map.ensure(ctx->m_total + 8);
        hipLaunchKernelGGL(mrf_map_kernel, dim3((unsigned)(((size_t)F * 16 + 255) / 256)), dim3(256), 0, s, ctx->r_ptr, ctx->r_view, ctx->r_adj_ptr, ctx->r_adj, F, ctx->m_edge.p, ctx->m_cls.p, ctx->m_map.p); MVS_LAUNCH_CHECK();
        ctx->pq.ensure(ctx->csr_nnz + 1);
    }
    ctx->m_msg_a.ensure(ctx->m_total + 1024);
    MVS_HIP(hipMemsetAsync(ctx->m_msg_a.p, 0, (ctx->m_total + 1024) * sizeof(msg_t), s));
    const size_t F1 = (size_t)F + 1;
    ctx->m_stride = (uint32_t)F1;
    ctx->m_sel.ensure(2 * F1); ctx->m_lab.ensure(2 * F1); ctx->m_cost.ensure(2 * F1);
    ctx->m_sel2.ensure(F1); ctx->m_cand.ensure(F1); ctx->m_gain.ensure(F1);
    MVS_HIP(hipMemsetAsync(ctx->m_sel.p, 0, 2 * F1 * sizeof(uint32_t), s));
    MVS_HIP(hipMemsetAsync(ctx->m_lab.p, 0, 2 * F1 * sizeof(uint32_t), s));
    MVS_HIP(hipMemsetAsync(ctx->m_cost.p, 0, 2 * F1 * sizeof(float), s));
    mvs_mrf_progress init; memset(&init, 0, sizeof(init)); init.best = ~0ull; init.energy = ~0ull; init.w = 0u; init.best_w = 1u;
    if (F && params->max_sweeps <= 0) {
        hipLaunchKernelGGL(mrf_argmin_unary_kernel, dim3(nb), dim3(256), 0, s, ctx->r_ptr, ctx->r_view, ctx->r_cost, F, ctx->m_sel.p, ctx->m_lab.p, ctx->m_cost.p);
        MVS_LAUNCH_CHECK();
        init.w = 1u; init.best_w = 0u;
    }
    ctx->b_sel = ctx->m_sel.p + init.best_w * F1; ctx->b_lab = ctx->m_lab.p + init.best_w * F1; ctx->b_cost = ctx->m_cost.p + init.best_w * F1;
    ctx->best_resolved = true;
    MVS_HIP(hipMemsetAsync(ctx->m_gain.p, 0, F1 * sizeof(float), s));
    const size_t epart = 4 + 2 * (size_t)EPART_BLOCKS * std::max<size_t>(ctx->m_colours, 1);
    ctx->m_energy.ensure(epart);
    MVS_HIP(hipMemsetAsync(ctx->m_energy.p, 0, epart * sizeof(unsigned long long), s));
    ctx->m_state.ensure(1); ctx->m_hist.ensure((size_t)std::max(params->max_sweeps, 0) + 2);
    ensure_report_ring(ctx);
    ctx->seq_base += ctx->steps_issued;
    ctx->h_ring[mvs_ctx::RING] = init;
    MVS_HIP(hipMemcpyAsync(ctx->m_state.p, &ctx->h_ring[mvs_ctx::RING], sizeof(init), hipMemcpyHostToDevice, s));
    ctx->m_ctl.ensure(4);
    uint32_t* stage = ctx->h_seq + (mvs_ctx::RING + mvs_ctx::ICM_RING);
    stage[0] = 0u; stage[1] = ctx->seq_base;
    MVS_HIP(hipMemcpyAsync(ctx->m_ctl.p, stage, 2 * sizeof(uint32_t), hipMemcpyHostToDevice, s));
    MVS_HIP(hipMemsetAsync(ctx->m_hist.p, 0xFF, sizeof(unsigned long long), s));
    ctx->steps_issued = 0; ctx->icm_dirty_valid = false; ctx->exact_valid = false;
}

void resolve_best(mvs_ctx* ctx) {
    if (ctx->best_resolved) return;
    if (!ctx->m_state.p) throw StatusError(MVS_ERR_STATE, "mrf setup first");
    mvs_mrf_progress p;
    static_assert(sizeof(p) % 4 == 0 && sizeof(p) <= 64, "mvs_mrf_progress travels through read_words");
    read_words(ctx, ctx->m_state.p, &p, (uint32_t)(sizeof(p) / 4));
    const size_t o = (size_t)(p.best_w & 1u) * ctx->m_stride;
    ctx->b_sel = ctx->m_sel.p + o; ctx->b_lab = ctx->m_lab.p + o; ctx->b_cost = ctx->m_cost.p + o;
    ctx->best_resolved = true;
}

void mrf_step(mvs_ctx* ctx, const unsigned long long* energy, const unsigned long long* const* peer_tab, uint32_t n_peer, uint32_t peer_off) {
    hipStream_t s = ctx->stream;
    const mvs_mrf_params& P = ctx->m_params;
    if (!ctx->h_ring) throw StatusError(MVS_ERR_STATE, "mrf step before mrf setup");
    const uint32_t n = ++ctx->steps_issued, slot = n % mvs_ctx::RING;
    const unsigned long long* partial = nullptr; uint32_t n_partial = 0;
    if (!energy && !peer_tab) { partial = ctx->m_energy.p + 4; n_partial = ctx->m_energy_from_sweep ? EPART_BLOCKS * std::max<uint32_t>(ctx->m_colours, 1u) : ctx->m_energy_blocks; }
    (void)n; (void)slot;
    hipLaunchKernelGGL(mrf_step_kernel, dim3(1), dim3(1024), 0, s, ctx->m_state.p, ctx->m_hist.p, energy, partial, n_partial, ctx->m_energy.p,
                       ctx->d_ring, ctx->d_seq, (uint32_t)mvs_ctx::RING, ctx->m_ctl.p, P.max_sweeps, P.min_sweeps, P.window, P.min_improvement, peer_tab, n_peer, peer_off);
    MVS_LAUNCH_CHECK();
    ctx->icm_dirty_valid = false; ctx->best_resolved = false; ctx->exact_valid = false;
}
void mrf_poll(mvs_ctx* ctx, uint32_t step, mvs_mrf_progress* out) {
    if (step == 0 || step > ctx->steps_issued || step + mvs_ctx::RING <= ctx->steps_issued)
        throw StatusError(MVS_ERR_INVALID, "mrf poll: step not among the last 16 issued");
    const uint32_t slot = step % mvs_ctx::RING;
    wait_report(ctx, slot, ctx->seq_base + step);
    *out = ctx->h_ring[slot];
}

void ensure_report_ring(mvs_ctx* ctx) {
    if (ctx->h_ring) return;
    constexpr uint32_t NS = mvs_ctx::RING + mvs_ctx::ICM_RING;
    MVS_HIP(hipHostMalloc((void**)&ctx->h_ring, (mvs_ctx::RING + 1) * sizeof(mvs_mrf_progress), hipHostMallocCoherent));
    MVS_HIP(hipHostGetDevicePointer((void**)&ctx->d_ring, ctx->h_ring, 0));
    MVS_HIP(hipHostMalloc((void**)&ctx->h_seq, (NS + 2) * sizeof(uint32_t), hipHostMallocCoherent));
    MVS_HIP(hipHostGetDevicePointer((void**)&ctx->d_seq, ctx->h_seq, 0));
    MVS_HIP(hipHostMalloc((void**)&ctx->h_icm, mvs_ctx::ICM_RING * sizeof(uint32_t), hipHostMallocCoherent));
    MVS_HIP(hipHostGetDevicePointer((void**)&ctx->d_icm, ctx->h_icm, 0));
    for (uint32_t k = 0; k < NS; ++k) ctx->h_seq[k] = 0u;
    ctx->seq_base = 1u; ctx->icm_seq = 0x40000000u;
}
void report_u32(mvs_ctx* ctx, const uint32_t* d_src, uint32_t* d_dst, uint32_t seq_slot, uint32_t seq) {
    hipLaunchKernelGGL(report_u32_kernel, dim3(1), dim3(1), 0, ctx->stream, d_src, d_dst, ctx->d_seq + seq_slot, seq);
    MVS_LAUNCH_CHECK();
}
void read_words(mvs_ctx* ctx, const void* d_src, void* out, uint32_t n_words) {
    if (n_words == 0 || n_words > 64) throw StatusError(MVS_ERR_INVALID, "read_words: 1 .. 64 words");
    if (!ctx->h_rb) {
        MVS_HIP(hipHostMalloc((void**)&ctx->h_rb, (128 + 1024) * sizeof(uint32_t), hipHostMallocCoherent));
        MVS_HIP(hipHostGetDevicePointer((void**)&ctx->d_rb, ctx->h_rb, 0));
        ctx->h_rb[64] = 0u; ctx->rb_seq = 0u;
    }
    const uint32_t seq = ++ctx->rb_seq ? ctx->rb_seq : ++ctx->rb_seq;
    hipLaunchKernelGGL(report_words_kernel, dim3(1), dim3(64), 0, ctx->stream, (const uint32_t*)d_src, n_words, ctx->d_rb, ctx->d_rb + 64, seq);
    MVS_LAUNCH_CHECK();
    const volatile uint32_t* p = ctx->h_rb + 64;
    for (uint64_t spins = 1; *p != seq; ++spins) {
        if ((spins & 0x3FFFu) == 0u) {
            const hipError_t q = hipStreamQuery(ctx->stream);
            if (q == hipSuccess) { if (*p == seq) break; throw HipError("a device read-back did not arrive although the stream is idle"); }
            if (q != hipErrorNotReady) MVS_HIP(q);
        }
        __builtin_ia32_pause();
    }
    std::atomic_thread_fence(std::memory_order_acquire);
    memcpy(out, ctx->h_rb, n_words * sizeof(uint32_t));
}
void read_block(mvs_ctx* ctx, const void* d_src, void* out, size_t bytes) {
    if (bytes <= 64 * sizeof(uint32_t) && bytes % 4 == 0) { read_words(ctx, d_src, out, (uint32_t)(bytes / 4)); return; }
    if (bytes > 1024 * sizeof(uint32_t)) throw StatusError(MVS_ERR_INVALID, "read_block: at most 4 KB");
    if (!ctx->h_rb) { uint32_t dummy; read_words(ctx, d_src, &dummy, 1); }
    MVS_HIP(hipMemcpyAsync(ctx->h_rb + 128, d_src, bytes, hipMemcpyDeviceToHost, ctx->stream));
    MVS_HIP(hipStreamSynchronize(ctx->stream));
    memcpy(out, ctx->h_rb + 128, bytes);
}
void wait_report(mvs_ctx* ctx, uint32_t seq_slot, uint32_t seq) {
    const volatile uint32_t* p = ctx->h_seq + seq_slot;
    for (uint64_t spins = 1; *p != seq; ++spins) {
        if ((spins & 0x3FFFu) == 0u) {
            const hipError_t q = hipStreamQuery(ctx->stream);
            if (q == hipSuccess) { if (*p == seq) break; throw HipError("a device report did not arrive although the stream is idle"); }
            if (q != hipErrorNotReady) MVS_HIP(q);
        }
        __builtin_ia32_pause();
    }
    std::atomic_thread_fence(std::memory_order_acquire);
}

static float sweep_alpha(const mvs_ctx* ctx) {
    const uint32_t p = (uint32_t)std::max(ctx->mrf_damp_period, 0);
    if (p == 0) return 0.0f;
    return (p == 1 || ctx->m_sweep_no % p == 1u) ? ctx->m_params.damping : 0.0f;
}

template <int G>
static unsigned launch_sweep4_g(mvs_ctx* ctx, uint32_t phase, uint32_t qb, uint32_t qe, unsigned slot, unsigned slot_cap) {
    constexpr int NPB = 256 / G;
    const unsigned need = (qe - qb + NPB - 1) / NPB;
    const float rho = ctx->m_params.rho, alpha = sweep_alpha(ctx);
    static std::atomic<int> resident_once{0};
    int resident = resident_once.load(std::memory_order_relaxed);
    if (resident == 0) {
        int per_cu = 0; hipDeviceProp_t prop;
        MVS_HIP(hipOccupancyMaxActiveBlocksPerMultiprocessor(&per_cu, mrf_sweep4_kernel<G, true, true, true>, 256, 0));
        MVS_HIP(hipGetDeviceProperties(&prop, ctx->device));
        resident = std::max(1, per_cu) * prop.multiProcessorCount;
        resident_once.store(resident, std::memory_order_relaxed);
    }
    unsigned blocks = ctx->mrf_blocks_per_cu > 0 ? 256u * (unsigned)ctx->mrf_blocks_per_cu : (unsigned)resident;
    blocks = std::max(1u, std::min(std::min(need, blocks), slot_cap));
    if (blocks > 8) blocks &= ~7u;
    msg_t* msg = reinterpret_cast<msg_t*>(ctx->m_msg_a.p);
    unsigned long long* partial = ctx->m_energy.p + 4 + 2 * ((size_t)EPART_BLOCKS * phase + slot);
#define SWEEP4_ARGS dim3(blocks), dim3(256), 0, ctx->stream, ctx->m_desc.p, ctx->m_rec.p, msg, ctx->m_state.p, ctx->m_lab.p, ctx->m_stride, qb, qe, rho, alpha, partial
    if (alpha != 0.0f) {
        if (ctx->mrf_late_old) { if (ctx->mrf_xcd) hipLaunchKernelGGL((mrf_sweep4_kernel<G, true, true, true>), SWEEP4_ARGS); else hipLaunchKernelGGL((mrf_sweep4_kernel<G, true, false, true>), SWEEP4_ARGS); }
        else { if (ctx->mrf_xcd) hipLaunchKernelGGL((mrf_sweep4_kernel<G, true, true, false>), SWEEP4_ARGS); else hipLaunchKernelGGL((mrf_sweep4_kernel<G, true, false, false>), SWEEP4_ARGS); }
    } else { if (ctx->mrf_xcd) hipLaunchKernelGGL((mrf_sweep4_kernel<G, false, true, false>), SWEEP4_ARGS); else hipLaunchKernelGGL((mrf_sweep4_kernel<G, false, false, false>), SWEEP4_ARGS); }
#undef SWEEP4_ARGS
    MVS_LAUNCH_CHECK();
    return blocks;
}
static unsigned launch_sweep8(mvs_ctx* ctx, uint32_t phase, uint32_t qb, uint32_t qe, unsigned slot, unsigned slot_cap) {
    constexpr int NPB = 256 / 8;
    const unsigned need = (qe - qb + NPB - 1) / NPB;
    const float rho = ctx->m_params.rho, alpha = sweep_alpha(ctx);
    static std::atomic<int> resident_once{0};
    int resident = resident_once.load(std::memory_order_relaxed);
    if (resident == 0) {
        int per_cu = 0; hipDeviceProp_t prop;
        MVS_HIP(hipOccupancyMaxActiveBlocksPerMultiprocessor(&per_cu, mrf_sweep8_kernel<true, true>, 256, 0));
        MVS_HIP(hipGetDeviceProperties(&prop, ctx->device));
        resident = std::max(1, per_cu) * prop.multiProcessorCount;
        resident_once.store(resident, std::memory_order_relaxed);
    }
    unsigned blocks = ctx->mrf_blocks_per_cu > 0 ? 256u * (unsigned)ctx->mrf_blocks_per_cu : (unsigned)resident;
    blocks = std::max(1u, std::min(std::min(need, blocks), slot_cap));
    if (blocks > 8) blocks &= ~7u;
    msg_t* msg = reinterpret_cast<msg_t*>(ctx->m_msg_a.p);
    unsigned long long* partial = ctx->m_energy.p + 4 + 2 * ((size_t)EPART_BLOCKS * phase + slot);
#define SWEEP8_ARGS dim3(blocks), dim3(256), 0, ctx->stream, ctx->m_desc.p, ctx->m_rec.p, msg, ctx->m_state.p, ctx->m_lab.p, ctx->m_stride, qb, qe, rho, alpha, partial
    if (alpha != 0.0f) { if (ctx->mrf_xcd) hipLaunchKernelGGL((mrf_sweep8_kernel<true, true>), SWEEP8_ARGS); else hipLaunchKernelGGL((mrf_sweep8_kernel<true, false>), SWEEP8_ARGS); }
    else { if (ctx->mrf_xcd) hipLaunchKernelGGL((mrf_sweep8_kernel<false, true>), SWEEP8_ARGS); else hipLaunchKernelGGL((mrf_sweep8_kernel<false, false>), SWEEP8_ARGS); }
#undef SWEEP8_ARGS
    MVS_LAUNCH_CHECK();
    return blocks;
}
static unsigned launch_sweep_generic(mvs_ctx* ctx, uint32_t phase, uint32_t qb, uint32_t qe, unsigned slot, unsigned slot_cap) {
    const unsigned need = qe - qb;
    const unsigned blocks = std::max(1u, std::min(std::min(need, 256u * 4u), slot_cap));
    const float rho = ctx->m_params.rho, alpha = sweep_alpha(ctx);
    msg_t* msg = reinterpret_cast<msg_t*>(ctx->m_msg_a.p);
    unsigned long long* partial = ctx->m_energy.p + 4 + 2 * ((size_t)EPART_BLOCKS * phase + slot);
#define GENERIC_ARGS dim3(blocks), dim3(256), 0, ctx->stream, ctx->r_ptr, ctx->r_view, ctx->r_cost, ctx->r_adj_ptr, ctx->r_adj, ctx->m_edge.p, ctx->m_map.p, ctx->m_colour.p, msg, ctx->m_perm.p, \
                     ctx->m_state.p, ctx->m_lab.p, ctx->m_stride, ctx->pq.p, qb, qe, rho, alpha, partial
    if (alpha != 0.0f) hipLaunchKernelGGL(mrf_sweep_generic_kernel<true>, GENERIC_ARGS);
    else hipLaunchKernelGGL(mrf_sweep_generic_kernel<false>, GENERIC_ARGS);
#undef GENERIC_ARGS
    MVS_LAUNCH_CHECK();
    return blocks;
}

static void sub_range(mvs_ctx* ctx, uint32_t sub, uint32_t zone, uint32_t nb0, uint32_t ne0, uint32_t* qb, uint32_t* qe) {
    const uint32_t key = 2u * sub + zone;
    const uint32_t cb = ctx->m_sub_begin[key], ce = ctx->m_sub_begin[key + 1];
    if (ce <= cb || (nb0 == 0 && ne0 >= ctx->csr_faces)) { *qb = cb; *qe = ce; return; }
    if (ctx->m_range_nb != nb0 || ctx->m_range_ne != ne0 || ctx->m_range_q.size() != 2 * (size_t)N_KEY) {
        uint32_t* d = ctx->m_sub.p + N_KEY + 2;
        hipLaunchKernelGGL(mrf_sub_range_kernel, dim3((N_KEY + 255) / 256), dim3(256), 0, ctx->stream, ctx->m_perm.p, ctx->m_sub.p, nb0, ne0, d);
        MVS_LAUNCH_CHECK();
        ctx->m_range_q.assign(2 * (size_t)N_KEY, 0);
        MVS_HIP(hipMemcpyAsync(ctx->m_range_q.data(), d, 2 * N_KEY * sizeof(uint32_t), hipMemcpyDeviceToHost, ctx->stream));
        MVS_HIP(hipStreamSynchronize(ctx->stream));
        ctx->m_range_nb = nb0; ctx->m_range_ne = ne0;
    }
    *qb = ctx->m_range_q[2 * key]; *qe = ctx->m_range_q[2 * key + 1];
}

void mrf_sweep_phase(mvs_ctx* ctx, uint32_t phase, uint32_t nb0, uint32_t ne0, int part) {
    if (phase == 0 && part != MRF_PART_INTERIOR) ++ctx->m_sweep_no;
    if (phase >= ctx->m_colours || ne0 <= nb0) return;
    constexpr unsigned EPART_BOUNDARY = 256;
    struct Launch { uint32_t g, qb, qe; } L[10]; int n = 0;
    for (uint32_t g = 0; g < 5; ++g) {
        const uint32_t sub = g < 4 ? 4 * phase + g : SUB_GENERIC + phase;
        uint32_t b0 = 0, b1 = 0, i0 = 0, i1 = 0;
        if (part != MRF_PART_INTERIOR) sub_range(ctx, sub, 0, nb0, ne0, &b0, &b1);
        if (part != MRF_PART_BOUNDARY) sub_range(ctx, sub, 1, nb0, ne0, &i0, &i1);
        if (b1 > b0 && i1 > i0 && b1 == i0) { L[n++] = {g, b0, i1}; continue; }
        if (b1 > b0) L[n++] = {g, b0, b1};
        if (i1 > i0) L[n++] = {g, i0, i1};
    }
    unsigned slot = part == MRF_PART_INTERIOR ? EPART_BOUNDARY : 0u;
    const unsigned slot_end = part == MRF_PART_BOUNDARY ? EPART_BOUNDARY : EPART_BLOCKS;
    for (int k = 0; k < n; ++k) {
        const unsigned cap = slot_end - slot - (unsigned)(n - 1 - k);
        const uint32_t qb = L[k].qb, qe = L[k].qe;
        switch (L[k].g) {
            case 0: slot += launch_sweep4_g<8>(ctx, phase, qb, qe, slot, cap); break;
            case 1: slot += ctx->m_wide_layout ? launch_sweep8(ctx, phase, qb, qe, slot, cap) : launch_sweep4_g<16>(ctx, phase, qb, qe, slot, cap); break;
            case 2: slot += launch_sweep4_g<32>(ctx, phase, qb, qe, slot, cap); break;
            case 3: slot += launch_sweep4_g<64>(ctx, phase, qb, qe, slot, cap); break;
            default: slot += launch_sweep_generic(ctx, phase, qb, qe, slot, cap);
        }
    }
}
void mrf_sweep(mvs_ctx* ctx, uint32_t nb0, uint32_t ne0) {
    for (uint32_t ph = 0; ph < ctx->m_colours; ++ph) mrf_sweep_phase(ctx, ph, nb0, ne0, MRF_PART_ALL);
    ctx->m_energy_from_sweep = nb0 == 0 && ne0 >= ctx->csr_faces && ctx->m_colours > 0;
}

__global__ void mrf_exact_cost_kernel(const uint32_t* __restrict__ col_ptr, const uint16_t* __restrict__ view_id, const float* __restrict__ cost,
                                      const uint32_t* __restrict__ lab, uint32_t node_begin, uint32_t node_end, uint32_t* __restrict__ sel, float* __restrict__ selcost,
                                      uint32_t* __restrict__ foreign ) {
    const uint32_t i = node_begin + blockIdx.x * blockDim.x + threadIdx.x;
    if (i >= node_end) return;
    const uint32_t p0 = col_ptr[i], K = col_ptr[i + 1] - p0, l = lab[i];
    const uint32_t t = (K && l) ? label_position(view_id, p0, K, l) : 0u;
    if ((K != 0u) != (l != 0u) || (K && l && (uint32_t)view_id[p0 + t] + 1u != l)) atomicAdd(foreign, 1u);
    sel[i] = t;
    selcost[i] = K ? cost[p0 + t] : 1.0f;
}
void mrf_exact_costs(mvs_ctx* ctx, uint32_t nb0, uint32_t ne0) {
    resolve_best(ctx);
    if (ne0 <= nb0) return;
    if (ctx->exact_valid && ctx->exact_nb == nb0 && ctx->exact_ne == ne0) return;
    ctx->exact_valid = true; ctx->exact_nb = nb0; ctx->exact_ne = ne0;
    MVS_HIP(hipMemsetAsync(ctx->m_moved.p + 6, 0, sizeof(uint32_t), ctx->stream));
    hipLaunchKernelGGL(mrf_exact_cost_kernel, dim3((ne0 - nb0 + 255) / 256), dim3(256), 0, ctx->stream, ctx->r_ptr, ctx->r_view, ctx->r_cost, (const uint32_t*)ctx->b_lab, nb0, ne0, ctx->b_sel, ctx->b_cost, ctx->m_moved.p + 6);
    MVS_LAUNCH_CHECK();
}

void mrf_energy(mvs_ctx* ctx, bool best, uint32_t nb0, uint32_t ne0, bool reduce) {
    const unsigned blocks = ne0 > nb0 ? std::min<unsigned>((ne0 - nb0 + 255) / 256, 2048u) : 0u;
    ctx->m_energy_blocks = blocks; ctx->m_energy_from_sweep = false;
    unsigned long long* partial = ctx->m_energy.p + 4;
    if (best) mrf_exact_costs(ctx, nb0, ne0);
    if (blocks) {
        if (best) hipLaunchKernelGGL(mrf_energy_kernel, dim3(blocks), dim3(256), 0, ctx->stream, ctx->r_ptr, ctx->r_view, ctx->r_cost, ctx->r_adj_ptr, ctx->r_adj, ctx->b_lab, ctx->b_cost, (const mvs_mrf_progress*)nullptr, 0u, nb0, ne0, partial);
        else hipLaunchKernelGGL(mrf_energy_kernel, dim3(blocks), dim3(256), 0, ctx->stream, ctx->r_ptr, ctx->r_view, ctx->r_cost, ctx->r_adj_ptr, ctx->r_adj, ctx->m_lab.p, ctx->m_cost.p, ctx->m_state.p, ctx->m_stride, nb0, ne0, partial);
        MVS_LAUNCH_CHECK();
    }
    if (!reduce) return;
    hipLaunchKernelGGL(mrf_energy_reduce_kernel, dim3(1), dim3(1024), 0, ctx->stream, partial, blocks, ctx->m_energy.p, (unsigned long long*)nullptr);
    MVS_LAUNCH_CHECK();
}
void mrf_sweep_energy_reduce(mvs_ctx* ctx, unsigned long long* out2) {
    const uint32_t n = EPART_BLOCKS * std::max<uint32_t>(ctx->m_colours, 1u);
    hipLaunchKernelGGL(mrf_energy_reduce_kernel, dim3(1), dim3(1024), 0, ctx->stream, ctx->m_energy.p + 4, n, ctx->m_energy.p, out2);
    MVS_LAUNCH_CHECK();
}

void mrf_keep_best(mvs_ctx* ctx) {
    ctx->icm_dirty_valid = false; ctx->best_resolved = false; ctx->exact_valid = false;
    if (!ctx->m_state.p) throw StatusError(MVS_ERR_STATE, "mrf setup first");
    hipLaunchKernelGGL(mrf_flip_kernel, dim3(1), dim3(1), 0, ctx->stream, ctx->m_state.p);
    MVS_LAUNCH_CHECK();
}

void mrf_icm_gain(mvs_ctx* ctx, uint32_t nb0, uint32_t ne0) {
    if (ne0 <= nb0) return;
    resolve_best(ctx);
    const uint32_t K = ctx->m_kmax, n = ne0 - nb0;
    const bool whole = nb0 == 0 && ne0 == ctx->csr_faces;
#define ICM_G(GG, B, E, LIST) hipLaunchKernelGGL(mrf_icm_gain_kernel<GG>, dim3(((E) - (B) + (256 / GG) - 1) / (256 / GG)), dim3(256), 0, ctx->stream, ctx->r_ptr, ctx->r_view, ctx->r_cost, \
                                     ctx->r_adj_ptr, ctx->r_adj, ctx->b_sel, ctx->b_lab, (B), (E), ctx->m_gain.p, ctx->m_cand.p, (LIST), (const uint32_t*)nullptr)
    if (whole && ctx->icm_dirty_valid) {
        const uint32_t* list = ctx->m_alist.p; const uint32_t* cnt = ctx->m_moved.p + 1;
#define ICM_L(GG) hipLaunchKernelGGL(mrf_icm_gain_kernel<GG>, dim3(std::max(1u, std::min<unsigned>((n + (256 / GG) - 1) / (256 / GG), 1024u))), dim3(256), 0, ctx->stream, ctx->r_ptr, ctx->r_view, ctx->r_cost, \
                                     ctx->r_adj_ptr, ctx->r_adj, ctx->b_sel, ctx->b_lab, 0u, 0u, ctx->m_gain.p, ctx->m_cand.p, list, cnt)
        if (K <= 8) ICM_L(8); else if (K <= 16) ICM_L(16); else if (K <= 32) ICM_L(32); else ICM_L(64);
#undef ICM_L
        MVS_LAUNCH_CHECK();
        return;
    }
    if (whole) {
        const uint32_t nf = ctx->m_n_fast;
        if (nf) {
#define ICM_D(GG) hipLaunchKernelGGL(mrf_icm_gain_desc_kernel<GG>, dim3(std::max(1u, std::min<unsigned>((nf + (256 / GG) - 1) / (256 / GG), 256u * 8u))), dim3(256), 0, ctx->stream, \
                                     ctx->m_desc.p, ctx->r_ptr, ctx->r_view, ctx->r_cost, ctx->b_sel, ctx->b_lab, 0u, nf, ctx->m_gain.p, ctx->m_cand.p)
            if (K <= 8) ICM_D(8); else if (K <= 64) ICM_D(16); else ICM_D(32);
#undef ICM_D
            MVS_LAUNCH_CHECK();
        }
        if (nf < n) ICM_G(64, nf, n, (const uint32_t*)ctx->m_perm.p);
    } else {
        const uint32_t* none = nullptr;
        if (K <= 8) ICM_G(8, nb0, ne0, none); else if (K <= 64) ICM_G(16, nb0, ne0, none); else if (K <= 128) ICM_G(32, nb0, ne0, none); else ICM_G(64, nb0, ne0, none);
    }
#undef ICM_G
    MVS_LAUNCH_CHECK();
    ctx->icm_dirty_valid = whole;
}
void mrf_icm_apply(mvs_ctx* ctx, uint32_t nb0, uint32_t ne0) {
    MVS_HIP(hipMemsetAsync(ctx->m_moved.p, 0, 2 * sizeof(uint32_t), ctx->stream));
    if (ne0 <= nb0) return;
    resolve_best(ctx);
    const bool whole = nb0 == 0 && ne0 == ctx->csr_faces;
    if (!whole) ctx->icm_dirty_valid = false;
    uint32_t* alist = nullptr;
    if (ctx->icm_dirty_valid) {
        ctx->m_alist.ensure((size_t)ctx->csr_faces + (size_t)ctx->m_n_adj + 16);
        alist = ctx->m_alist.p;
    }
    hipLaunchKernelGGL(mrf_icm_apply_kernel, dim3((ne0 - nb0 + 255) / 256), dim3(256), 0, ctx->stream, ctx->r_ptr, ctx->r_view, ctx->r_cost, ctx->r_adj_ptr, ctx->r_adj,
                       ctx->m_gain.p, ctx->m_cand.p, ctx->b_sel, ctx->b_lab, ctx->b_cost, nb0, ne0, ctx->m_moved.p, alist, ctx->t_perm);
    MVS_LAUNCH_CHECK();
}
void mrf_labels(mvs_ctx* ctx, uint32_t nb0, uint32_t ne0, uint32_t* d_labels, uint32_t out[2], bool caller_order) {
    uint32_t* bu = ctx->m_moved.p + 2;
    resolve_best(ctx);
    MVS_HIP(hipMemsetAsync(bu, 0, 2 * sizeof(uint32_t), ctx->stream));
    if (ne0 > nb0) {
        const uint32_t* foreign = (ctx->exact_valid && ctx->exact_nb == nb0 && ctx->exact_ne == ne0) ? ctx->m_moved.p + 6 : (const uint32_t*)nullptr;
        hipLaunchKernelGGL(mrf_labels_kernel, dim3((ne0 - nb0 + 255) / 256), dim3(256), 0, ctx->stream, ctx->b_lab, nb0, ne0, ctx->csr_views, d_labels, bu, caller_order ? ctx->t_perm : (const uint32_t*)nullptr, foreign);
        MVS_LAUNCH_CHECK();
    }
    read_words(ctx, bu, out, 2);
}

}
```

mvs-texturing_amd/csrc/mgpu.hip:

```cpp
#include "ctx.h"
#include "../../include/mvs_viewsel_blocks.h"
#include <vector>

namespace mvs {
void mrf_setup(mvs_ctx* ctx, const mvs_mrf_params* params);
void mrf_sweep(mvs_ctx* ctx, uint32_t nb0, uint32_t ne0);
void mrf_energy(mvs_ctx* ctx, bool best, uint32_t nb0, uint32_t ne0, bool reduce = true);
void mrf_keep_best(mvs_ctx* ctx);
void mrf_sweep_phase(mvs_ctx* ctx, uint32_t phase, uint32_t nb0, uint32_t ne0, int part = MRF_PART_ALL);
void mrf_step(mvs_ctx* ctx, const unsigned long long* energy, const unsigned long long* const* peer_tab = nullptr, uint32_t n_peer = 0, uint32_t peer_off = 0);
void mrf_poll(mvs_ctx* ctx, uint32_t step, mvs_mrf_progress* out);
void mrf_icm_gain(mvs_ctx* ctx, uint32_t nb0, uint32_t ne0);
void mrf_icm_apply(mvs_ctx* ctx, uint32_t nb0, uint32_t ne0);
void mrf_labels(mvs_ctx* ctx, uint32_t nb0, uint32_t ne0, uint32_t* d_labels, uint32_t out[2], bool caller_order = false);
void resolve_best(mvs_ctx* ctx);
void set_adjacency(mvs_ctx* ctx, const uint32_t* adj_ptr, const uint32_t* adj, int on_device, bool table_order);
mvs_status api_fail(mvs_status st, const std::string& msg);

namespace {
__global__ void gather_kernel(const uint32_t* __restrict__ src, const mvs_mrf_progress* __restrict__ st, uint32_t buf_stride, const uint32_t* __restrict__ idx, uint64_t n, uint32_t* __restrict__ dst) {
    if (st) src += (size_t)st->w * buf_stride;
    for (uint64_t k = (uint64_t)blockIdx.x * blockDim.x + threadIdx.x; k < n; k += (uint64_t)gridDim.x * blockDim.x) dst[k] = src[idx[k]];
}
__global__ void scatter_kernel(uint32_t* __restrict__ dst, const mvs_mrf_progress* __restrict__ st, uint32_t buf_stride, const uint32_t* __restrict__ idx, uint64_t n, const uint32_t* __restrict__ src) {
    if (st) dst += (size_t)st->w * buf_stride;
    for (uint64_t k = (uint64_t)blockIdx.x * blockDim.x + threadIdx.x; k < n; k += (uint64_t)gridDim.x * blockDim.x) dst[idx[k]] = src[k];
}
__global__ void gather_msg_kernel(const uint8_t* __restrict__ src, const uint32_t* __restrict__ idx, uint64_t n, uint32_t* __restrict__ dst) {
    for (uint64_t k = (uint64_t)blockIdx.x * blockDim.x + threadIdx.x; k < n; k += (uint64_t)gridDim.x * blockDim.x) dst[k] = src[idx[k]];
}
__global__ void scatter_msg_kernel(uint8_t* __restrict__ dst, const uint32_t* __restrict__ idx, uint64_t n, const uint32_t* __restrict__ src) {
    for (uint64_t k = (uint64_t)blockIdx.x * blockDim.x + threadIdx.x; k < n; k += (uint64_t)gridDim.x * blockDim.x) dst[idx[k]] = (uint8_t)src[k];
}
__global__ void gather2_kernel(const uint8_t* __restrict__ a, const uint32_t* __restrict__ b, const mvs_mrf_progress* __restrict__ st, uint32_t buf_stride, const uint32_t* __restrict__ idx, uint64_t n, uint32_t* __restrict__ dst) {
    b += (size_t)st->w * buf_stride;
    for (uint64_t k = (uint64_t)blockIdx.x * blockDim.x + threadIdx.x; k < n; k += (uint64_t)gridDim.x * blockDim.x) {
        const uint32_t i = idx[k];
        dst[k] = (i & 0x80000000u) ? b[i & 0x7FFFFFFFu] : a[i];
    }
}
__global__ void scatter2_kernel(uint8_t* __restrict__ a, uint32_t* __restrict__ b, const mvs_mrf_progress* __restrict__ st, uint32_t buf_stride, const uint32_t* __restrict__ idx, uint64_t n, const uint32_t* __restrict__ src) {
    b += (size_t)st->w * buf_stride;
    for (uint64_t k = (uint64_t)blockIdx.x * blockDim.x + threadIdx.x; k < n; k += (uint64_t)gridDim.x * blockDim.x) {
        const uint32_t i = idx[k];
        if (i & 0x80000000u) b[i & 0x7FFFFFFFu] = src[k]; else a[i] = (uint8_t)src[k];
    }
}
__global__ void counts_kernel(const uint32_t* __restrict__ col_ptr, uint32_t n, uint32_t* __restrict__ counts) {
    const uint32_t i = blockIdx.x * blockDim.x + threadIdx.x;
    if (i < n) counts[i] = col_ptr[i + 1] - col_ptr[i];
}
}

static uint8_t* mrf_msg(mvs_ctx* ctx) { return ctx->m_msg_a.p; }
static uint32_t* mrf_array(mvs_ctx* ctx, int which, const mvs_mrf_progress** st) {
    *st = nullptr;
    switch (which) {
        case MVS_MRF_LAB: *st = ctx->m_state.p; return ctx->m_lab.p;
        case MVS_MRF_GAIN: return (uint32_t*)ctx->m_gain.p;
        case MVS_MRF_BEST_LAB: resolve_best(ctx); return ctx->b_lab;
    }
    throw StatusError(MVS_ERR_INVALID, "bad array selector");
}
}

using namespace mvs;

#define MVS_API_BEGIN try { MVS_HIP(hipSetDevice(ctx->device));
#define MVS_API_END                                                               \
    } catch (const StatusError& e) { return api_fail(e.st, e.what()); }           \
      catch (const HipError& e) { return api_fail(MVS_ERR_HIP, e.what()); }       \
      catch (const std::exception& e) { return api_fail(MVS_ERR_HIP, e.what()); } \
    return MVS_OK;

extern "C" {

mvs_status mvs_ctx_dc_get_max(mvs_ctx* ctx, float* dst) {
    if (!ctx || !dst) return api_fail(MVS_ERR_INVALID, "null argument");
    if (ctx->dc_phase < 1) return api_fail(MVS_ERR_STATE, "dc_phase1 first");
    MVS_API_BEGIN
    MVS_HIP(hipMemcpyAsync(dst, ctx->max_q.p, sizeof(float), hipMemcpyDeviceToDevice, ctx->stream));
    MVS_API_END
}
mvs_status mvs_ctx_dc_set_max(mvs_ctx* ctx, const float* src) {
    if (!ctx || !src) return api_fail(MVS_ERR_INVALID, "null argument");
    if (ctx->dc_phase < 1) return api_fail(MVS_ERR_STATE, "dc_phase1 first");
    MVS_API_BEGIN
    MVS_HIP(hipMemcpyAsync(ctx->max_q.p, src, sizeof(float), hipMemcpyDeviceToDevice, ctx->stream));
    MVS_API_END
}
mvs_status mvs_ctx_dc_get_histogram(mvs_ctx* ctx, uint32_t* dst) {
    if (!ctx || !dst) return api_fail(MVS_ERR_INVALID, "null argument");
    if (ctx->dc_phase < 2) return api_fail(MVS_ERR_STATE, "dc_phase2 first");
    MVS_API_BEGIN
    MVS_HIP(hipMemcpyAsync(dst, ctx->hist.p, MVS_HIST_WORDS * sizeof(uint32_t), hipMemcpyDeviceToDevice, ctx->stream));
    MVS_API_END
}
mvs_status mvs_ctx_dc_set_histogram(mvs_ctx* ctx, const uint32_t* src) {
    if (!ctx || !src) return api_fail(MVS_ERR_INVALID, "null argument");
    if (ctx->dc_phase < 2) return api_fail(MVS_ERR_STATE, "dc_phase2 first");
    MVS_API_BEGIN
    MVS_HIP(hipMemcpyAsync(ctx->hist.p, src, MVS_HIST_WORDS * sizeof(uint32_t), hipMemcpyDeviceToDevice, ctx->stream));
    MVS_API_END
}

mvs_status mvs_ctx_costs_export(mvs_ctx* ctx, uint32_t* counts, uint16_t* view_id, float* cost) {
    if (!ctx || !counts) return api_fail(MVS_ERR_INVALID, "null argument");
    if (!ctx->have_costs) return api_fail(MVS_ERR_STATE, "no data costs on the device");
    MVS_API_BEGIN
    const uint32_t F = ctx->csr_faces;
    if (F) { hipLaunchKernelGGL(counts_kernel, dim3((F + 255) / 256), dim3(256), 0, ctx->stream, ctx->r_ptr, F, counts); MVS_LAUNCH_CHECK(); }
    if (ctx->csr_nnz && view_id) MVS_HIP(hipMemcpyAsync(view_id, ctx->r_view, ctx->csr_nnz * sizeof(uint16_t), hipMemcpyDeviceToDevice, ctx->stream));
    if (ctx->csr_nnz && cost) MVS_HIP(hipMemcpyAsync(cost, ctx->r_cost, ctx->csr_nnz * sizeof(float), hipMemcpyDeviceToDevice, ctx->stream));
    MVS_API_END
}

mvs_status mvs_ctx_mrf_setup(mvs_ctx* ctx, const uint32_t* adj_ptr, const uint32_t* adj, int adj_on_device, const mvs_mrf_params* params) {
    if (!ctx || !adj_ptr || !adj) return api_fail(MVS_ERR_INVALID, "null argument");
    if (!ctx->have_costs) return api_fail(MVS_ERR_STATE, "mrf setup needs data costs");
    MVS_API_BEGIN
    mvs_mrf_params P; if (params) P = *params; else mvs_mrf_default_params(&P);
    set_adjacency(ctx, adj_ptr, adj, adj_on_device, false);
    mrf_setup(ctx, &P);
    MVS_API_END
}

mvs_status mvs_ctx_mrf_sweep(mvs_ctx* ctx, uint32_t nb0, uint32_t ne0) {
    if (!ctx || nb0 > ne0 || ne0 > ctx->csr_faces) return api_fail(MVS_ERR_INVALID, "bad node range");
    MVS_API_BEGIN
    Prof pr(ctx, "mrf_sweep");
    mrf_sweep(ctx, nb0, ne0);
    MVS_API_END
}

mvs_status mvs_ctx_mrf_sweep_phase(mvs_ctx* ctx, uint32_t phase, uint32_t nb0, uint32_t ne0) {
    if (!ctx || nb0 > ne0 || ne0 > ctx->csr_faces || phase >= ctx->m_colours) return api_fail(MVS_ERR_INVALID, "bad phase or node range");
    MVS_API_BEGIN
    Prof pr(ctx, "mrf_sweep");
    mrf_sweep_phase(ctx, phase, nb0, ne0);
    MVS_API_END
}
mvs_status mvs_ctx_mrf_setup_marked(mvs_ctx* ctx, const uint32_t* adj_ptr, const uint32_t* adj, int adj_on_device, const mvs_mrf_params* params, const uint8_t* marks_device) {
    if (!ctx || !adj_ptr || !adj) return api_fail(MVS_ERR_INVALID, "null argument");
    if (!ctx->have_costs) return api_fail(MVS_ERR_STATE, "mrf setup needs data costs");
    MVS_API_BEGIN
    mvs_mrf_params P; if (params) P = *params; else mvs_mrf_default_params(&P);
    set_adjacency(ctx, adj_ptr, adj, adj_on_device, false);
    struct Marks { mvs_ctx* c; ~Marks() { c->m_bnd = nullptr; } } marks{ctx};
    ctx->m_bnd = marks_device;
    mrf_setup(ctx, &P);
    MVS_API_END
}
mvs_status mvs_ctx_mrf_sweep_phase_part(mvs_ctx* ctx, uint32_t phase, uint32_t nb0, uint32_t ne0, int part) {
    if (!ctx || nb0 > ne0 || ne0 > ctx->csr_faces || phase >= ctx->m_colours || part < 0 || part > 2) return api_fail(MVS_ERR_INVALID, "bad phase, node range or part");
    MVS_API_BEGIN
    Prof pr(ctx, part == MRF_PART_BOUNDARY ? "mrf_sweep_boundary" : "mrf_sweep");
    mrf_sweep_phase(ctx, phase, nb0, ne0, part);
    MVS_API_END
}
mvs_status mvs_ctx_mrf_layout(mvs_ctx* ctx, uint32_t* in_off_host, uint64_t n_edges) {
    if (!ctx || (n_edges && !in_off_host)) return api_fail(MVS_ERR_INVALID, "null argument");
    MVS_API_BEGIN
    if (n_edges) MVS_HIP(hipMemcpy2DAsync(in_off_host, sizeof(uint32_t), ctx->m_edge.p, sizeof(MrfEdge), sizeof(uint32_t), n_edges, hipMemcpyDeviceToHost, ctx->stream));
    MVS_HIP(hipStreamSynchronize(ctx->stream));
    MVS_API_END
}

mvs_status mvs_ctx_mrf_gather(mvs_ctx* ctx, int which, const uint32_t* idx, uint64_t n, void* dst) {
    if (!ctx || (n && (!idx || !dst))) return api_fail(MVS_ERR_INVALID, "null argument");
    MVS_API_BEGIN
    if (n && which == MVS_MRF_MSG_LAB) {
        if (ctx->m_total >= 0x80000000ull) throw StatusError(MVS_ERR_UNSUPPORTED, "combined addressing needs < 2^31 message words");
        hipLaunchKernelGGL(gather2_kernel, dim3((unsigned)std::min<uint64_t>((n + 255) / 256, 4096)), dim3(256), 0, ctx->stream, mrf_msg(ctx), ctx->m_lab.p, ctx->m_state.p, ctx->m_stride, idx, n, (uint32_t*)dst);
        MVS_LAUNCH_CHECK();
    } else if (n && which == MVS_MRF_MSG) {
        hipLaunchKernelGGL(gather_msg_kernel, dim3((unsigned)std::min<uint64_t>((n + 255) / 256, 4096)), dim3(256), 0, ctx->stream, mrf_msg(ctx), idx, n, (uint32_t*)dst);
        MVS_LAUNCH_CHECK();
    } else if (n) {
        const mvs_mrf_progress* st; const uint32_t* arr = mrf_array(ctx, which, &st);
        hipLaunchKernelGGL(gather_kernel, dim3((unsigned)std::min<uint64_t>((n + 255) / 256, 4096)), dim3(256), 0, ctx->stream, arr, st, ctx->m_stride, idx, n, (uint32_t*)dst);
        MVS_LAUNCH_CHECK();
    }
    MVS_API_END
}
mvs_status mvs_ctx_mrf_scatter(mvs_ctx* ctx, int which, const uint32_t* idx, uint64_t n, const void* src) {
    if (!ctx || (n && (!idx || !src))) return api_fail(MVS_ERR_INVALID, "null argument");
    MVS_API_BEGIN
    if (n) { ctx->icm_dirty_valid = false; ctx->exact_valid = false; }
    if (n && which == MVS_MRF_MSG_LAB) {
        hipLaunchKernelGGL(scatter2_kernel, dim3((unsigned)std::min<uint64_t>((n + 255) / 256, 4096)), dim3(256), 0, ctx->stream, mrf_msg(ctx), ctx->m_lab.p, ctx->m_state.p, ctx->m_stride, idx, n, (const uint32_t*)src);
        MVS_LAUNCH_CHECK();
    } else if (n && which == MVS_MRF_MSG) {
        hipLaunchKernelGGL(scatter_msg_kernel, dim3((unsigned)std::min<uint64_t>((n + 255) / 256, 4096)), dim3(256), 0, ctx->stream, mrf_msg(ctx), idx, n, (const uint32_t*)src);
        MVS_LAUNCH_CHECK();
    } else if (n) {
        const mvs_mrf_progress* st; uint32_t* arr = mrf_array(ctx, which, &st);
        hipLaunchKernelGGL(scatter_kernel, dim3((unsigned)std::min<uint64_t>((n + 255) / 256, 4096)), dim3(256), 0, ctx->stream, arr, st, ctx->m_stride, idx, n, (const uint32_t*)src);
        MVS_LAUNCH_CHECK();
    }
    MVS_API_END
}

mvs_status mvs_ctx_mrf_energy(mvs_ctx* ctx, int which_sel, uint32_t nb0, uint32_t ne0, uint64_t* dst) {
    if (!ctx || !dst || nb0 > ne0 || ne0 > ctx->csr_faces) return api_fail(MVS_ERR_INVALID, "bad argument");
    if (which_sel != MVS_MRF_LAB && which_sel != MVS_MRF_BEST_LAB) return api_fail(MVS_ERR_INVALID, "energy: LAB or BEST_LAB");
    MVS_API_BEGIN
    mrf_energy(ctx, which_sel == MVS_MRF_BEST_LAB, nb0, ne0);
    MVS_HIP(hipMemcpyAsync(dst, ctx->m_energy.p, 2 * sizeof(uint64_t), hipMemcpyDeviceToDevice, ctx->stream));
    MVS_API_END
}

mvs_status mvs_ctx_mrf_keep_best(mvs_ctx* ctx) {
    if (!ctx) return api_fail(MVS_ERR_INVALID, "ctx is null");
    MVS_API_BEGIN
    mrf_keep_best(ctx);
    MVS_API_END
}

mvs_status mvs_ctx_mrf_step(mvs_ctx* ctx, const uint64_t* energy_device) {
    if (!ctx) return api_fail(MVS_ERR_INVALID, "ctx is null");
    MVS_API_BEGIN
    mrf_step(ctx, (const unsigned long long*)energy_device);
    MVS_API_END
}
mvs_status mvs_ctx_mrf_poll(mvs_ctx* ctx, uint32_t step, mvs_mrf_progress* out) {
    if (!ctx || !out) return api_fail(MVS_ERR_INVALID, "null argument");
    MVS_API_BEGIN
    mrf_poll(ctx, step, out);
    MVS_API_END
}

mvs_status mvs_ctx_mrf_icm_gain(mvs_ctx* ctx, uint32_t nb0, uint32_t ne0) {
    if (!ctx || nb0 > ne0 || ne0 > ctx->csr_faces) return api_fail(MVS_ERR_INVALID, "bad node range");
    MVS_API_BEGIN
    mrf_icm_gain(ctx, nb0, ne0);
    MVS_API_END
}
mvs_status mvs_ctx_mrf_icm_apply(mvs_ctx* ctx, uint32_t nb0, uint32_t ne0, uint32_t* moved) {
    if (!ctx || !moved || nb0 > ne0 || ne0 > ctx->csr_faces) return api_fail(MVS_ERR_INVALID, "bad argument");
    MVS_API_BEGIN
    mrf_icm_apply(ctx, nb0, ne0);
    MVS_HIP(hipMemcpyAsync(moved, ctx->m_moved.p, sizeof(uint32_t), hipMemcpyDeviceToDevice, ctx->stream));
    MVS_API_END
}

mvs_status mvs_ctx_mrf_labels(mvs_ctx* ctx, uint32_t nb0, uint32_t ne0, uint32_t* labels, uint32_t* unseen_out) {
    if (!ctx || !labels || nb0 > ne0 || ne0 > ctx->csr_faces) return api_fail(MVS_ERR_INVALID, "bad argument");
    MVS_API_BEGIN
    uint32_t bu[2];
    mrf_labels(ctx, nb0, ne0, labels, bu);
    if (unseen_out) *unseen_out = bu[1];
    if (bu[0]) throw StatusError(MVS_ERR_LABELING, "Incorrect labeling");
    MVS_API_END
}

}
```

mvs-texturing_amd/viewsel.py:

```python
import ctypes as C
import os

import numpy as np

_HERE = os.path.dirname(os.path.abspath(__file__))
_LIB_PATH = os.environ.get("MVS_VIEWSEL_LIB") or os.path.join(_HERE, "csrc", "libmvs_viewsel.so")
_BLOCKS_PATH = os.path.join(_HERE, "csrc", "libmvs_blocks.so")


class MvsError(RuntimeError):
    def __init__(self, status, message):
        super().__init__("%s (status %d)" % (message, status))
        self.status = status


class CMesh(C.Structure):
    _fields_ = [("n_verts", C.c_uint32), ("n_faces", C.c_uint32), ("verts", C.c_void_p), ("faces", C.c_void_p),
                ("face_normals", C.c_void_p)]


class CView(C.Structure):
    _fields_ = [("pos", C.c_float * 3), ("viewdir", C.c_float * 3), ("K", C.c_float * 9), ("w2c", C.c_float * 16),
                ("width", C.c_int32), ("height", C.c_int32), ("rgb", C.c_void_p)]


class Settings(C.Structure):
    _fields_ = [("data_term", C.c_int32), ("outlier_removal", C.c_int32), ("geometric_visibility_test", C.c_int32)]

    DATA_TERMS = {"area": 0, "gmi": 1}
    OUTLIER = {"none": 0, "gauss_damping": 1, "gauss_clamping": 2}

    def __init__(self, data_term="gmi", outlier_removal="none", geometric_visibility_test=True):
        super().__init__(self.DATA_TERMS[data_term] if isinstance(data_term, str) else int(data_term),
                         self.OUTLIER[outlier_removal] if isinstance(outlier_removal, str) else int(outlier_removal),
                         1 if geometric_visibility_test else 0)


class CCsr(C.Structure):
    _fields_ = [("n_faces", C.c_uint32), ("n_views", C.c_uint32), ("nnz", C.c_uint64), ("col_ptr", C.c_void_p),
                ("view_id", C.c_void_p), ("cost", C.c_void_p)]


class MrfParams(C.Structure):
    _fields_ = [("max_sweeps", C.c_int32), ("min_sweeps", C.c_int32), ("window", C.c_int32),
                ("min_improvement", C.c_float), ("damping", C.c_float), ("rho", C.c_float), ("icm_iters", C.c_int32),
                ("region_rounds", C.c_int32)]


class MrfStats(C.Structure):
    _fields_ = [("energy_fixed", C.c_uint64), ("energy", C.c_double), ("cut_edges", C.c_uint64), ("sweeps", C.c_uint32),
                ("icm_iters", C.c_uint32), ("unseen", C.c_uint32), ("region_rounds", C.c_uint32), ("region_moves", C.c_uint32)]


class MrfProgress(C.Structure):
    _fields_ = [("sweep", C.c_uint32), ("stopped", C.c_uint32), ("improved", C.c_uint32), ("stop_sweep", C.c_uint32),
                ("energy", C.c_uint64), ("best", C.c_uint64), ("w", C.c_uint32), ("best_w", C.c_uint32)]


class Subgraphs(C.Structure):
    _fields_ = [("n_faces", C.c_uint32), ("n_labels", C.c_uint32), ("n_components", C.c_uint32),
                ("label_ptr", C.c_void_p), ("comp_ptr", C.c_void_p), ("comp_faces", C.c_void_p)]


class DcStats(C.Structure):
    _fields_ = [(n, C.c_uint64) for n in ("pairs", "cull_backface", "cull_angle", "cull_outside", "cull_occluded",
                                           "cull_zero_quality", "nnz_pre", "nnz", "rays", "ray_nodes", "ray_tris", "ray_packets", "ray_packets_generic")] + \
               [("max_quality", C.c_float), ("percentile", C.c_float), ("footprints_lane_group", C.c_uint64), ("footprints_rewalked", C.c_uint64), ("ray_leaf_rounds", C.c_uint64)]


def _stats_dict(s):
    return {f[0]: getattr(s, f[0]) for f in s._fields_}


def lib_path():
    return _LIB_PATH


def blocks_lib_path():
    return _BLOCKS_PATH


BLOCK_SYMBOLS = frozenset((
    "mvs_ctx_dc_get_max", "mvs_ctx_dc_set_max", "mvs_ctx_dc_get_histogram", "mvs_ctx_dc_set_histogram", "mvs_ctx_costs_export",
    "mvs_ctx_mrf_setup", "mvs_ctx_mrf_setup_marked", "mvs_ctx_mrf_sweep", "mvs_ctx_mrf_sweep_phase", "mvs_ctx_mrf_sweep_phase_part", "mvs_ctx_mrf_layout", "mvs_ctx_mrf_gather", "mvs_ctx_mrf_scatter",
    "mvs_ctx_mrf_energy", "mvs_ctx_mrf_keep_best", "mvs_ctx_mrf_step", "mvs_ctx_mrf_poll", "mvs_ctx_mrf_icm_gain", "mvs_ctx_mrf_icm_apply",
    "mvs_ctx_mrf_labels"))


_lib = None


def load_library():
    global _lib
    if _lib is not None:
        return _lib
    try:
        import torch
    except ImportError:
        pass
    if not os.path.exists(_LIB_PATH):
        raise MvsError(-1, "HIP library %s is missing: run `python mvs-texturing_amd/build.py` "
                           "(or __graft_entry__.build()); there is no CPU fallback" % _LIB_PATH)
    L = C.CDLL(_LIB_PATH)
    L.mvs_last_error.restype = C.c_char_p
    L.mvs_status_string.restype = C.c_char_p
    L.mvs_last_call_profile.restype = C.c_char_p
    vp, u32, u64, i32 = C.c_void_p, C.c_uint32, C.c_uint64, C.c_int
    sig = {
        "mvs_mrf_default_params": [C.POINTER(MrfParams)], "mvs_default_settings": [C.POINTER(Settings)],
        "mvs_data_costs": [C.POINTER(CMesh), C.POINTER(CView), u32, C.POINTER(Settings), C.POINTER(CCsr), C.POINTER(DcStats)],
        "mvs_csr_free": [C.POINTER(CCsr)], "mvs_subgraphs_free": [C.POINTER(Subgraphs)],
        "mvs_view_selection": [C.POINTER(CCsr), vp, vp, C.POINTER(MrfParams), vp, C.POINTER(MrfStats)],
        "mvs_write_spt": [C.POINTER(CCsr), C.c_char_p], "mvs_read_spt": [C.c_char_p, C.POINTER(CCsr)],
        "mvs_write_labeling_vec": [vp, u32, C.c_char_p],
        "mvs_prepare_mesh": [u32, vp, u32, vp, vp, vp, C.POINTER(u32)],
        "mvs_build_adjacency_graph": [u32, u32, vp, vp, C.POINTER(vp), C.POINTER(u64)],
        "mvs_ctx_build_adjacency": [vp, C.POINTER(vp), C.POINTER(vp), C.POINTER(u64)],
        "mvs_get_subgraphs": [u32, vp, vp, vp, u32, C.POINTER(Subgraphs)],
        "mvs_ctx_get_subgraphs": [vp, u32, vp, vp, i32, vp, i32, u32, C.POINTER(Subgraphs), i32],
        "mvs_ctx_create": [i32, C.POINTER(vp)], "mvs_ctx_destroy": [vp], "mvs_ctx_set_stream": [vp, vp],
        "mvs_ctx_synchronize": [vp], "mvs_set_option": [vp, C.c_char_p, C.c_int64],
        "mvs_ctx_get_profile": [vp, C.c_char_p, C.c_size_t],
        "mvs_scene_set_mesh": [vp, C.POINTER(CMesh), i32], "mvs_scene_set_views": [vp, C.POINTER(CView), u32, i32],
        "mvs_scene_set_face_range": [vp, u32, u32],
        "mvs_ctx_data_costs": [vp, C.POINTER(Settings), C.POINTER(DcStats)],
        "mvs_ctx_dc_phase1": [vp, C.POINTER(Settings)], "mvs_ctx_dc_get_max": [vp, vp], "mvs_ctx_dc_set_max": [vp, vp],
        "mvs_ctx_dc_phase2": [vp], "mvs_ctx_dc_get_histogram": [vp, vp], "mvs_ctx_dc_set_histogram": [vp, vp],
        "mvs_ctx_dc_phase3": [vp, C.POINTER(DcStats)],
        "mvs_ctx_costs_device": [vp, C.POINTER(CCsr)], "mvs_ctx_costs_download": [vp, C.POINTER(CCsr), C.POINTER(vp)],
        "mvs_ctx_costs_upload": [vp, C.POINTER(CCsr), i32], "mvs_ctx_costs_export": [vp, vp, vp, vp],
        "mvs_ctx_view_selection": [vp, vp, vp, i32, C.POINTER(MrfParams), vp, i32, C.POINTER(MrfStats)],
        "mvs_ctx_mrf_setup": [vp, vp, vp, i32, C.POINTER(MrfParams)], "mvs_ctx_mrf_sweep": [vp, u32, u32],
        "mvs_ctx_mrf_setup_marked": [vp, vp, vp, i32, C.POINTER(MrfParams), vp], "mvs_ctx_mrf_sweep_phase_part": [vp, u32, u32, u32, i32],
        "mvs_ctx_mrf_num_phases": [vp, C.POINTER(u32)], "mvs_ctx_mrf_diagnostics": [vp, C.POINTER(u32)], "mvs_ctx_mrf_sweep_phase": [vp, u32, u32, u32], "mvs_ctx_mrf_layout": [vp, vp, u64],
        "mvs_ctx_mrf_gather": [vp, i32, vp, u64, vp], "mvs_ctx_mrf_scatter": [vp, i32, vp, u64, vp],
        "mvs_ctx_mrf_energy": [vp, i32, u32, u32, vp], "mvs_ctx_mrf_keep_best": [vp],
        "mvs_ctx_mrf_step": [vp, vp], "mvs_ctx_mrf_poll": [vp, u32, C.POINTER(MrfProgress)],
        "mvs_ctx_mrf_icm_gain": [vp, u32, u32], "mvs_ctx_mrf_icm_apply": [vp, u32, u32, vp],
        "mvs_ctx_mrf_labels": [vp, u32, u32, vp, C.POINTER(u32)],
        "mvs_ctx_prune_labels": [vp, u32], "mvs_undistort_image": [vp, C.c_int32, C.c_int32, C.c_float, C.c_float, C.c_float, vp],
        "mvs_postprocess_face_infos": [u32, u32, vp, vp, vp, vp, C.POINTER(Settings), C.POINTER(CCsr), C.POINTER(DcStats)],
        "mvs_comm_unique_id": [vp], "mvs_comm_create_rccl": [i32, i32, i32, vp, C.POINTER(vp)], "mvs_comm_create_local": [i32, C.POINTER(vp)], "mvs_comm_create_local_devices": [i32, vp, C.POINTER(vp)],
        "mvs_comm_info": [vp, C.POINTER(i32), C.POINTER(i32), C.POINTER(i32)],
        "mvs_comm_destroy": [vp], "mvs_comm_abort": [vp], "mvs_shard_create": [vp, vp, vp, vp, vp, C.POINTER(vp)], "mvs_shard_destroy": [vp],
        "mvs_shard_data_costs": [vp, C.POINTER(Settings), C.POINTER(DcStats), C.POINTER(u64)],
        "mvs_shard_view_selection": [vp, C.POINTER(MrfParams), vp, C.POINTER(MrfStats)],
        "mvs_shard_plan_info": [vp, C.POINTER(u64), C.POINTER(u64), C.POINTER(C.c_double)],
        "mvs_shard_transport_info": [vp, C.POINTER(i32), C.POINTER(u64), C.POINTER(i32), C.POINTER(u32)],
        "mvs_shard_own_faces": [vp, vp, C.POINTER(u32)],
        "mvs_ctx_partition_faces": [vp, i32, vp, vp], "mvs_partition_faces": [C.POINTER(CMesh), i32, vp, vp],
        "mvs_ctx_table_order": [vp, vp, C.POINTER(i32)],
        "mvs_data_costs_stream": [C.POINTER(CMesh), C.POINTER(CView), u32, C.POINTER(Settings), vp, vp, C.POINTER(CCsr), C.POINTER(DcStats)],
        "mvs_view_selection_cached": [u64, u32, u32, u64, vp, vp, C.POINTER(MrfParams), vp, C.POINTER(MrfStats)],
    }
    blocks = None
    if os.path.exists(_BLOCKS_PATH):
        try:
            blocks = C.CDLL(_BLOCKS_PATH, mode=C.RTLD_GLOBAL)
        except OSError:
            blocks = None
    L._blocks_declared = []
    for name, argtypes in sig.items():
        if name in BLOCK_SYMBOLS:
            if blocks is None:
                continue
            fn = getattr(blocks, name)
            setattr(L, name, fn)
            L._blocks_declared.append(name)
        else:
            fn = getattr(L, name)
        fn.argtypes = argtypes
        if name not in ("mvs_mrf_default_params", "mvs_default_settings", "mvs_csr_free", "mvs_subgraphs_free", "mvs_ctx_destroy", "mvs_comm_destroy", "mvs_comm_abort", "mvs_shard_destroy"):
            fn.restype = C.c_int
    L._declared = sorted([k for k in sig.keys() if k not in BLOCK_SYMBOLS] + ["mvs_last_error", "mvs_status_string"])
    L._blocks = blocks
    _lib = L
    return L


def _check(L, st):
    if st != 0:
        raise MvsError(st, L.mvs_last_error().decode() or L.mvs_status_string(st).decode())


def _is_torch(a):
    return type(a).__module__.startswith("torch")


class DevArray:
    is_cuda = True

    def __init__(self, ptr, n):
        self.ptr, self.shape = int(ptr or 0), (int(n),)

    def data_ptr(self):
        return self.ptr

    def is_contiguous(self):
        return True


def _ptr(a):
    if a is None:
        return None, 0
    if _is_torch(a) or isinstance(a, DevArray):
        assert a.is_contiguous()
        return C.c_void_p(a.data_ptr()), 1 if a.is_cuda else 0
    assert a.flags["C_CONTIGUOUS"]
    return a.ctypes.data_as(C.c_void_p), 0


def default_mrf_params(**kw):
    p = MrfParams()
    load_library().mvs_mrf_default_params(C.byref(p))
    for k, v in kw.items():
        setattr(p, k, v)
    return p


class DataCosts:

    def __init__(self, n_faces, n_views, col_ptr, view_id, cost, quality=None):
        self.n_faces, self.n_views = int(n_faces), int(n_views)
        self.col_ptr, self.view_id, self.cost, self.quality = col_ptr, view_id, cost, quality

    cols = property(lambda self: self.n_faces)
    rows = property(lambda self: self.n_views)

    @property
    def nnz(self):
        return int(self.col_ptr[-1])

    def col(self, i):
        a, b = int(self.col_ptr[i]), int(self.col_ptr[i + 1])
        return list(zip(self.view_id[a:b].tolist(), self.cost[a:b].tolist()))

    def _struct(self):
        s = CCsr(self.n_faces, self.n_views, self.nnz, 0, 0, 0)
        s.col_ptr, dev0 = _ptr(self.col_ptr)
        s.view_id, dev1 = _ptr(self.view_id)
        s.cost, dev2 = _ptr(self.cost)
        assert dev0 == dev1 == dev2
        return s, dev0

    def save_to_file(self, path):
        L = load_library()
        s, dev = self._struct()
        assert not dev, "download first"
        _check(L, L.mvs_write_spt(C.byref(s), path.encode()))


class Context:

    def __init__(self, device=0):
        self.L = load_library()
        h = C.c_void_p()
        _check(self.L, self.L.mvs_ctx_create(device, C.byref(h)))
        self.h = h
        self.device = int(device)
        self._keep = {}

    def close(self):
        if getattr(self, "h", None):
            self.L.mvs_ctx_destroy(self.h)
            self.h = None

    __del__ = close

    def set_stream(self, stream_handle):
        _check(self.L, self.L.mvs_ctx_set_stream(self.h, C.c_void_p(stream_handle)))

    def synchronize(self):
        _check(self.L, self.L.mvs_ctx_synchronize(self.h))

    def set_option(self, name, value):
        _check(self.L, self.L.mvs_set_option(self.h, name.encode(), int(value)))

    def get_profile(self):
        import json
        buf = C.create_string_buffer(1 << 16)
        _check(self.L, self.L.mvs_ctx_get_profile(self.h, buf, len(buf)))
        return json.loads(buf.value.decode())

    def set_mesh(self, verts, faces, normals):
        pv, d0 = _ptr(verts); pf, d1 = _ptr(faces); pn, d2 = _ptr(normals)
        assert d0 == d1 == d2
        m = CMesh(int(verts.shape[0]), int(faces.shape[0]), pv, pf, pn)
        self._keep["mesh"] = (verts, faces, normals)
        self.n_faces = int(faces.shape[0])
        _check(self.L, self.L.mvs_scene_set_mesh(self.h, C.byref(m), d0))

    def set_views(self, cams, images):
# ... 196 lines not shown
```

Before: 76.05 million.

## Use per-face view bitmaps for MRF setup identity and rank lookups

```diff
diff --git a/include/mvs_viewsel_blocks.h b/include/mvs_viewsel_blocks.h
--- a/include/mvs_viewsel_blocks.h
+++ b/include/mvs_viewsel_blocks.h
@@ -21,6 +21,7 @@
 mvs_status mvs_ctx_mrf_sweep_phase_part(mvs_ctx* ctx, uint32_t phase, uint32_t node_begin, uint32_t node_end, int part);
 mvs_status mvs_ctx_mrf_sweep(mvs_ctx* ctx, uint32_t node_begin, uint32_t node_end);
 mvs_status mvs_ctx_mrf_layout(mvs_ctx* ctx, uint32_t* in_off_host, uint64_t n_edges);
+mvs_status mvs_ctx_mrf_tables(mvs_ctx* ctx, int which, void* dst_host, uint64_t cap_bytes, uint64_t* bytes_out);
 mvs_status mvs_ctx_mrf_gather(mvs_ctx* ctx, int which, const uint32_t* idx_device, uint64_t n, void* dst_device);
 mvs_status mvs_ctx_mrf_scatter(mvs_ctx* ctx, int which, const uint32_t* idx_device, uint64_t n, const void* src_device);
 mvs_status mvs_ctx_mrf_energy(mvs_ctx* ctx, int which_sel, uint32_t node_begin, uint32_t node_end, uint64_t* dst_device);
diff --git a/mvs-texturing_amd/csrc/api.hip b/mvs-texturing_amd/csrc/api.hip
--- a/mvs-texturing_amd/csrc/api.hip
+++ b/mvs-texturing_amd/csrc/api.hip
@@ -368,6 +368,8 @@
     else if (n == "shard_peer_push") ctx->shard_peer_push = value != 0;
     else if (n == "mrf_force_generic") ctx->mrf_force_generic = value != 0;
     else if (n == "mrf_wide") ctx->mrf_wide = value != 0;
+    else if (n == "mrf_setup_bitmap") ctx->mrf_setup_bitmap = value != 0;
+    else if (n == "mrf_bitmap_cap") ctx->mrf_bitmap_cap = (int)std::max<int64_t>(0, std::min<int64_t>(value, 32));
     else if (n == "mrf_graph") ctx->mrf_graph = value != 0;
     else if (n == "mrf_late_old") ctx->mrf_late_old = (int)value;
     else if (n == "mrf_damp_period") ctx->mrf_damp_period = (int)std::max<int64_t>(0, std::min<int64_t>(value, 64));
diff --git a/mvs-texturing_amd/csrc/ctx.h b/mvs-texturing_amd/csrc/ctx.h
--- a/mvs-texturing_amd/csrc/ctx.h
+++ b/mvs-texturing_amd/csrc/ctx.h
@@ -215,6 +215,10 @@
     int mrf_force_generic = 0;
     int mrf_wide = 1;
     bool m_wide_layout = false;
+    int mrf_setup_bitmap = 1;
+    int mrf_bitmap_cap = 32;
+    mvs::DBuf<uint32_t> m_bm;
+    uint32_t m_bm_words = 0;
     uint32_t m_range_nb = 0, m_range_ne = 0; std::vector<uint32_t> m_range_q;
     uint32_t m_sweep_no = 0;
     mvs_mrf_params m_params{};
diff --git a/mvs-texturing_amd/csrc/k_mrf.hip b/mvs-texturing_amd/csrc/k_mrf.hip
--- a/mvs-texturing_amd/csrc/k_mrf.hip
+++ b/mvs-texturing_amd/csrc/k_mrf.hip
@@ -343,6 +343,52 @@
     return lo < K ? lo : K - 1u;
 }
 
+constexpr uint32_t BM_MAX_WORDS = 32;
+__device__ __forceinline__ void wave_lds_order() { __builtin_amdgcn_fence(__ATOMIC_SEQ_CST, "wavefront"); __builtin_amdgcn_wave_barrier(); }
+__device__ __forceinline__ void or_runs_into(uint32_t* tile, uint32_t wd, uint32_t b, uint32_t gl) {
+#pragma unroll
+    for (uint32_t off = 1; off < 16; off <<= 1) {
+        const uint32_t w2 = __shfl_down(wd, off, 16), b2 = __shfl_down(b, off, 16);
+        if (gl + off < 16 && w2 == wd) b |= b2;
+    }
+    const uint32_t wp = __shfl_up(wd, 1, 16);
+    if (wd != 0xFFFFFFFFu && (gl == 0 || wp != wd)) atomicOr(&tile[wd], b);
+}
+__global__ void __launch_bounds__(256) mrf_bitmap_kernel(const uint32_t* __restrict__ col_ptr, const uint16_t* __restrict__ view_id, uint32_t F, uint32_t W,
+                                                         uint32_t* __restrict__ bm, uint32_t* __restrict__ unfit) {
+    __shared__ uint32_t s_b[16][BM_MAX_WORDS];
+    const uint32_t i = (blockIdx.x * blockDim.x + threadIdx.x) >> 4;
+    const uint32_t gl = threadIdx.x & 15;
+    if (i >= F) return;
+    uint32_t* tile = s_b[threadIdx.x >> 4];
+    tile[gl] = 0u; tile[gl + 16] = 0u;
+    wave_lds_order();
+    const uint32_t p0 = col_ptr[i], K = col_ptr[i + 1] - p0, nbits = 32u * W;
+    bool bad = false;
+    for (uint32_t tb = 0; tb < K; tb += 64) {
+        uint32_t v[4], pv[4];
+#pragma unroll
+        for (uint32_t k = 0; k < 4; ++k) {
+            const uint32_t t = tb + gl + 16u * k;
+            v[k] = t < K ? (uint32_t)view_id[p0 + t] : 0u;
+            pv[k] = (t < K && t > 0) ? (uint32_t)view_id[p0 + t - 1] : 0xFFFFFFFFu;
+        }
+#pragma unroll
+        for (uint32_t k = 0; k < 4; ++k) {
+            const bool on = tb + gl + 16u * k < K, in = on && v[k] < nbits;
+            if (on && !in) bad = true;
+            if (on && pv[k] != 0xFFFFFFFFu && pv[k] >= v[k]) bad = true;
+            or_runs_into(tile, in ? v[k] >> 5 : 0xFFFFFFFFu, in ? 1u << (v[k] & 31u) : 0u, gl);
+        }
+    }
+    wave_lds_order();
+    if (gl < W / 4u) {
+        const uint4 w4 = make_uint4(tile[4 * gl], tile[4 * gl + 1], tile[4 * gl + 2], tile[4 * gl + 3]);
+        *reinterpret_cast<uint4*>(bm + (size_t)i * W + 4 * gl) = w4;
+    }
+    if (bad) atomicOr(unfit, 1u);
+}
+
 __global__ void __launch_bounds__(256) mrf_ident_kernel(const uint32_t* __restrict__ col_ptr, const uint16_t* __restrict__ view_id, const uint32_t* __restrict__ adj_ptr,
                                                         const uint32_t* __restrict__ adj, uint32_t F, const MrfEdge* __restrict__ edge, const uint8_t* __restrict__ cls,
                                                         uint8_t* __restrict__ ident) {
@@ -374,36 +420,60 @@
         if (gl < 3 && e + gl < e1 && kj[gl] != 0u) ident[e + gl] = (uint8_t)((same >> gl) & 1u);
     }
 }
-__global__ void mrf_recsize_kernel(const uint32_t* __restrict__ col_ptr, const uint32_t* __restrict__ adj_ptr, const MrfEdge* __restrict__ edge,
-                                   const uint8_t* __restrict__ ident, const uint8_t* __restrict__ cls, const uint32_t* __restrict__ perm, uint32_t F, uint32_t wide,
-                                   uint32_t* __restrict__ rsz, uint32_t* __restrict__ qpos) {
+template <bool BM>
+__global__ void mrf_recsize_kernel(const uint32_t* __restrict__ col_ptr, const uint32_t* __restrict__ adj_ptr, const uint32_t* __restrict__ adj, const MrfEdge* __restrict__ edge,
+                                   uint8_t* __restrict__ ident, const uint32_t* __restrict__ bm, uint32_t W, const uint8_t* __restrict__ cls, const uint32_t* __restrict__ perm,
+                                   uint32_t F, uint32_t wide, uint32_t* __restrict__ rsz, uint32_t* __restrict__ qpos) {
     const uint32_t q = blockIdx.x * blockDim.x + threadIdx.x;
     if (q > F) return;
     uint32_t w = 0;
     if (q < F) {
         const uint32_t i = perm[q], K = col_ptr[i + 1] - col_ptr[i];
         qpos[i] = q;
-        if (K && cls[i] != CLS_GENERIC) {
+        const bool fast = K && cls[i] != CLS_GENERIC;
+        if (fast || BM) {
             w = (K + 3u) & ~3u;
             const bool w8 = wide != 0u && cls[i] == 1u;
             const uint32_t e0 = adj_ptr[i], e1 = adj_ptr[i + 1];
             for (uint32_t eb = e0; eb < e1; eb += 4) {
                 uint32_t kj[4], id[4];
 #pragma unroll
-                for (int t = 0; t < 4; ++t) { const bool on = eb + t < e1; kj[t] = on ? edge[eb + t].kj : 0u; id[t] = on ? ident[eb + t] : 1u; }
+                for (int t = 0; t < 4; ++t) { const bool on = eb + t < e1; kj[t] = on ? edge[eb + t].kj : 0u; id[t] = (on && !BM) ? ident[eb + t] : 1u; }
+                if (BM) {
+                    uint32_t j[4];
+#pragma unroll
+                    for (int t = 0; t < 4; ++t) { id[t] = (fast && kj[t] != 0u && kj[t] == K) ? 1u : 0u; j[t] = (id[t] != 0u) ? adj[eb + t] : i; }
+                    const uint4* a = reinterpret_cast<const uint4*>(bm + (size_t)i * W);
+                    if (id[0] | id[1] | id[2] | id[3]) {
+                        for (uint32_t w4 = 0; w4 < W / 4u; ++w4) {
+                            const uint4 x = a[w4];
+#pragma unroll
+                            for (int t = 0; t < 4; ++t) {
+                                const uint4 y = reinterpret_cast<const uint4*>(bm + (size_t)j[t] * W)[w4];
+                                if ((x.x ^ y.x) | (x.y ^ y.y) | (x.z ^ y.z) | (x.w ^ y.w)) id[t] = 0u;
+                            }
+                        }
+                    }
+#pragma unroll
+                    for (int t = 0; t < 4; ++t) if (eb + t < e1) ident[eb + t] = (uint8_t)id[t];
+                    if (!fast) continue;
+                }
 #pragma unroll
                 for (int t = 0; t < 4; ++t) if (kj[t] && !id[t]) w += w8 ? 2u * ((kj[t] + 7u) >> 3) : (kj[t] + 3u) >> 2;
             }
-            w = (w + 3u) & ~3u;
+            w = fast ? (w + 3u) & ~3u : 0u;
         }
     }
     rsz[q] = w;
 }
+template <bool RANK>
 __global__ void __launch_bounds__(256) mrf_record_kernel(const uint32_t* __restrict__ col_ptr, const uint16_t* __restrict__ view_id, const float* __restrict__ cost,
                                                          const uint32_t* __restrict__ adj_ptr, const uint32_t* __restrict__ adj, const MrfEdge* __restrict__ edge,
                                                          const uint8_t* __restrict__ ident, const uint8_t* __restrict__ cls, const uint32_t* __restrict__ qpos, const uint32_t* __restrict__ roff,
                                                          uint32_t F, uint32_t wide, uint32_t* __restrict__ rec) {
-    __shared__ uint16_t s_l[16][256];
+    __shared__ uint16_t s_l[16][RANK ? 1 : 256];
+    __shared__ uint32_t s_bits[16][RANK ? BM_MAX_WORDS : 1];
+    __shared__ uint8_t s_first[16][RANK ? BM_MAX_WORDS : 1];
     const uint32_t i = (blockIdx.x * blockDim.x + threadIdx.x) >> 4;
     const uint32_t gl = threadIdx.x & 15;
     if (i >= F) return;
@@ -415,6 +485,9 @@
     const uint32_t lmask = w8 ? 7u : 3u, lshift = w8 ? 3u : 2u;
     const uint32_t q = qpos[i];
     uint16_t* tile = s_l[threadIdx.x >> 4];
+    uint32_t* bits = s_bits[threadIdx.x >> 4];
+    uint8_t* first = s_first[threadIdx.x >> 4];
+    if (RANK) { bits[gl] = 0u; bits[gl + 16] = 0u; wave_lds_order(); }
     uint32_t* out = rec + REC_BASE + roff[q];
     const uint32_t K4 = (K + 3u) & ~3u;
     const uint32_t e0 = adj_ptr[i], deg = adj_ptr[i + 1] - e0;
@@ -426,10 +499,32 @@
 #pragma unroll
         for (uint32_t d = 0; d < 3; ++d) { kj3[d] = (kj[d] != 0u && idn[d] == 0u) ? kj[d] : 0u; q03[d] = col_ptr[nb[d]]; }
     }
-    for (uint32_t t = gl; t < K4; t += 16) {
-        uint32_t w = 0u;
-        if (t < K) { const uint32_t v = view_id[p0 + t]; tile[t] = (uint16_t)v; w = (cost_code(cost[p0 + t]) << 16) | v; }
-        out[t] = w;
+    if (!RANK) {
+        for (uint32_t t = gl; t < K4; t += 16) {
+            uint32_t w = 0u;
+            if (t < K) { const uint32_t v = view_id[p0 + t]; tile[t] = (uint16_t)v; w = (cost_code(cost[p0 + t]) << 16) | v; }
+            out[t] = w;
+        }
+    } else {
+        for (uint32_t tb = 0; tb < K4; tb += 64) {
+            uint32_t v[4], pv[4]; float cs[4];
+#pragma unroll
+            for (uint32_t k = 0; k < 4; ++k) {
+                const uint32_t t = tb + gl + 16u * k;
+                v[k] = t < K ? (uint32_t)view_id[p0 + t] : 0u;
+                cs[k] = t < K ? cost[p0 + t] : 0.0f;
+                pv[k] = (t < K && t > 0) ? (uint32_t)view_id[p0 + t - 1] : 0xFFFFFFFFu;
+            }
+#pragma unroll
+            for (uint32_t k = 0; k < 4; ++k) {
+                const uint32_t t = tb + gl + 16u * k;
+                const bool in = t < K && v[k] < 32u * BM_MAX_WORDS;
+                or_runs_into(bits, in ? v[k] >> 5 : 0xFFFFFFFFu, in ? 1u << (v[k] & 31u) : 0u, gl);
+                if (in && (pv[k] >> 5) != (v[k] >> 5)) first[v[k] >> 5] = (uint8_t)t;
+                if (t < K4) out[t] = t < K ? (cost_code(cs[k]) << 16) | v[k] : 0u;
+            }
+        }
+        wave_lds_order();
     }
     uint32_t pos = K4;
 #pragma unroll
@@ -441,6 +536,19 @@
             uint32_t key[4], lo[4] = {0u, 0u, 0u, 0u};
 #pragma unroll
             for (uint32_t r = 0; r < 4; ++r) { const uint32_t t2 = 4u * wI + r; key[r] = (t2 < kj) ? (uint32_t)view_id[q0 + t2] : 0xFFFFFFFFu; }
+            if (RANK) {
+                uint32_t word = 0u;
+#pragma unroll
+                for (uint32_t r = 0; r < 4; ++r) {
+                    const uint32_t v = key[r], wd = v < 32u * BM_MAX_WORDS ? v >> 5 : 0u;
+                    const uint32_t b = v < 32u * BM_MAX_WORDS ? bits[wd] : 0u, below = b & ((1u << (v & 31u)) - 1u);
+                    const uint32_t at = (uint32_t)first[wd] + __popc(below);
+                    const uint32_t byte = ((b >> (v & 31u)) & 1u) ? (at & lmask) * rs + (at >> lshift) : none_byte;
+                    word |= byte << (8 * r);
+                }
+                out[pos + wI] = word;
+                continue;
+            }
             for (uint32_t n = K; n > 1u;) {
                 const uint32_t half = n >> 1;
 #pragma unroll
@@ -1076,6 +1184,12 @@
     ctx->m_cls.ensure((size_t)F + 4);
     ctx->m_rev.ensure((size_t)E + 2);
     if (F) { hipLaunchKernelGGL(mrf_size_kernel, dim3(nb), dim3(256), 0, s, ctx->r_ptr, ctx->r_adj_ptr, ctx->r_adj, F, (uint32_t)(ctx->mrf_run_pad == 16 ? 15 : (ctx->mrf_wide ? 7 : 3)), force_generic, ctx->m_size.p, ctx->m_cls.p, maxes, ctx->m_rev.p); MVS_LAUNCH_CHECK(); }
+    const uint32_t bm_w = (ctx->csr_views + 31u) / 32u;
+    ctx->m_bm_words = (F && ctx->mrf_setup_bitmap && !force_generic && bm_w >= 1u && bm_w <= (uint32_t)ctx->mrf_bitmap_cap) ? (bm_w + 3u) & ~3u : 0u;
+    if (ctx->m_bm_words) {
+        ctx->m_bm.ensure((size_t)F * ctx->m_bm_words + 4);
+        hipLaunchKernelGGL(mrf_bitmap_kernel, dim3((unsigned)(((size_t)F * 16 + 255) / 256)), dim3(256), 0, s, ctx->r_ptr, ctx->r_view, F, ctx->m_bm_words, ctx->m_bm.p, maxes + 3); MVS_LAUNCH_CHECK();
+    }
     ctx->m_colour.ensure((size_t)F + 2); ctx->m_perm.ensure((size_t)F + 2); ctx->m_tmp_a.ensure((size_t)MAX_LAYOUT_COLOURS * ((size_t)F + 1) + 72); ctx->m_tmp_b.ensure((size_t)MAX_LAYOUT_COLOURS * ((size_t)F + 1) + 2); ctx->m_tmp_c.ensure((size_t)F + 2);
     ctx->m_colours = 0; ctx->m_sub_begin.assign(N_KEY + 1, 0); ctx->m_n_fast = 0; ctx->m_range_q.clear(); ctx->m_range_nb = ctx->m_range_ne = 0;
     ctx->m_sweep_no = 0;
@@ -1124,12 +1238,13 @@
         hipLaunchKernelGGL(mrf_inoff_kernel, dim3(nb), dim3(256), 0, s, ctx->m_perm.p, ctx->m_colour.p, ctx->r_adj_ptr, ctx->r_adj, ctx->m_size.p, ctx->m_rev.p, ctx->m_tmp_b.p, F, n_col, in_off.p); MVS_LAUNCH_CHECK();
         MVS_HIP(hipMemcpyAsync(maxes + 2, ctx->m_tmp_b.p + (n_ent - 1), sizeof(uint32_t), hipMemcpyDeviceToDevice, s));
     } else MVS_HIP(hipMemsetAsync(maxes + 2, 0, sizeof(uint32_t), s));
-    { uint32_t hm[3]; read_words(ctx, maxes, hm, 3); h[1] = hm[0]; h[2] = hm[1]; h[0] = hm[2]; }
+    { uint32_t hm[4]; read_words(ctx, maxes, hm, 4); h[1] = hm[0]; h[2] = hm[1]; h[0] = hm[2]; if (hm[3]) ctx->m_bm_words = 0; }
     ctx->m_total = (uint64_t)MSG_BASE + h[0]; ctx->m_kmax = h[1]; ctx->m_degmax = h[2];
     if (ctx->m_total >= 0xFFFFFFF0ull) throw StatusError(MVS_ERR_UNSUPPORTED, "message array exceeds 2^32 elements");
     if (F) { hipLaunchKernelGGL(mrf_edge_kernel, dim3(nb), dim3(256), 0, s, ctx->r_ptr, ctx->r_adj_ptr, ctx->r_adj, F, in_off.p, ctx->m_size.p, ctx->m_rev.p, ctx->m_edge.p); MVS_LAUNCH_CHECK(); }
     ctx->m_ident.ensure((size_t)E + 1);
-    MVS_HIP(hipMemsetAsync(ctx->m_ident.p, 0, (size_t)E + 1, s));
+    const bool bm = ctx->m_bm_words != 0;
+    if (!bm || !ctx->m_n_fast) MVS_HIP(hipMemsetAsync(ctx->m_ident.p, 0, (size_t)E + 1, s));
     ctx->m_fast = true;
     ctx->m_wide_layout = ctx->mrf_wide != 0;
     const uint32_t n_fast = ctx->m_n_fast, n_generic = F - n_fast;
@@ -1137,11 +1252,12 @@
         const size_t rec_cap = (size_t)REC_BASE + ctx->csr_nnz + 8 * (size_t)F + ctx->m_total / 4 + (ctx->mrf_wide ? (size_t)ctx->m_n_adj : 0) + 1024;
         ctx->m_rec.ensure(rec_cap);
         MVS_HIP(hipMemsetAsync(ctx->m_rec.p, 0, REC_BASE * sizeof(uint32_t), s));
-        hipLaunchKernelGGL(mrf_ident_kernel, dim3((unsigned)(((size_t)F * 16 + 255) / 256)), dim3(256), 0, s, ctx->r_ptr, ctx->r_view, ctx->r_adj_ptr, ctx->r_adj, F, ctx->m_edge.p, ctx->m_cls.p, ctx->m_ident.p); MVS_LAUNCH_CHECK();
+        if (!bm) { hipLaunchKernelGGL(mrf_ident_kernel, dim3((unsigned)(((size_t)F * 16 + 255) / 256)), dim3(256), 0, s, ctx->r_ptr, ctx->r_view, ctx->r_adj_ptr, ctx->r_adj, F, ctx->m_edge.p, ctx->m_cls.p, ctx->m_ident.p); MVS_LAUNCH_CHECK(); }
         uint32_t* rsz = ctx->m_tmp_a.p; uint32_t* roff = ctx->m_tmp_b.p;
-        hipLaunchKernelGGL(mrf_recsize_kernel, dim3((F + 256) / 256), dim3(256), 0, s, ctx->r_ptr, ctx->r_adj_ptr, ctx->m_edge.p, ctx->m_ident.p, ctx->m_cls.p, ctx->m_perm.p, F, (uint32_t)(ctx->mrf_wide ? 1 : 0), rsz, ctx->m_tmp_c.p); MVS_LAUNCH_CHECK();
+        hipLaunchKernelGGL(bm ? mrf_recsize_kernel<true> : mrf_recsize_kernel<false>, dim3((F + 256) / 256), dim3(256), 0, s, ctx->r_ptr, ctx->r_adj_ptr, ctx->r_adj, ctx->m_edge.p, ctx->m_ident.p,
+                           (const uint32_t*)ctx->m_bm.p, ctx->m_bm_words, ctx->m_cls.p, ctx->m_perm.p, F, (uint32_t)(ctx->mrf_wide ? 1 : 0), rsz, ctx->m_tmp_c.p); MVS_LAUNCH_CHECK();
         exclusive_scan_u32(ctx, rsz, roff, (size_t)F + 1, nullptr);
-        hipLaunchKernelGGL(mrf_record_kernel, dim3((unsigned)(((size_t)F * 16 + 255) / 256)), dim3(256), 0, s, ctx->r_ptr, ctx->r_view, ctx->r_cost, ctx->r_adj_ptr, ctx->r_adj,
+        hipLaunchKernelGGL(bm ? mrf_record_kernel<true> : mrf_record_kernel<false>, dim3((unsigned)(((size_t)F * 16 + 255) / 256)), dim3(256), 0, s, ctx->r_ptr, ctx->r_view, ctx->r_cost, ctx->r_adj_ptr, ctx->r_adj,
                            ctx->m_edge.p, ctx->m_ident.p, ctx->m_cls.p, ctx->m_tmp_c.p , roff, F, (uint32_t)(ctx->mrf_wide ? 1 : 0), ctx->m_rec.p); MVS_LAUNCH_CHECK();
         ctx->m_desc.ensure((size_t)F + 1);
         hipLaunchKernelGGL(mrf_desc_kernel, dim3((n_fast + 255) / 256), dim3(256), 0, s, ctx->r_ptr, ctx->r_adj_ptr, ctx->r_adj, ctx->m_edge.p, ctx->m_ident.p, ctx->m_perm.p, ctx->m_colour.p, roff, n_fast, ctx->m_desc.p); MVS_LAUNCH_CHECK();
@@ -1185,6 +1301,26 @@
     ctx->steps_issued = 0; ctx->icm_dirty_valid = false; ctx->exact_valid = false;
 }
 
+uint64_t mrf_tables(mvs_ctx* ctx, int which, void* dst, uint64_t cap) {
+    hipStream_t s = ctx->stream;
+    const uint32_t F = ctx->csr_faces, n_fast = ctx->m_n_fast;
+    uint64_t bytes = 0; const void* src = nullptr;
+    if (which == 0 || which == 1) {
+        if (n_fast) {
+            if (which == 0) { uint32_t total = 0; read_words(ctx, ctx->m_tmp_b.p + F, &total, 1); bytes = ((uint64_t)REC_BASE + total) * 4; src = ctx->m_rec.p; }
+            else { bytes = ((uint64_t)F + 1) * 4; src = ctx->m_tmp_b.p; }
+        }
+    } else if (which == 2) { bytes = (uint64_t)n_fast * sizeof(NodeDesc); src = ctx->m_desc.p; }
+    else if (which == 3) { bytes = ctx->m_n_adj; src = ctx->m_ident.p; }
+    else if (which == 4) { bytes = (uint64_t)F * ctx->m_bm_words * 4; src = ctx->m_bm.p; }
+    else throw StatusError(MVS_ERR_INVALID, "bad table selector");
+    if (dst && bytes && cap) {
+        MVS_HIP(hipMemcpyAsync(dst, src, std::min(bytes, cap), hipMemcpyDeviceToHost, s));
+        MVS_HIP(hipStreamSynchronize(s));
+    }
+    return bytes;
+}
+
 void resolve_best(mvs_ctx* ctx) {
     if (ctx->best_resolved) return;
     if (!ctx->m_state.p) throw StatusError(MVS_ERR_STATE, "mrf setup first");
@@ -1410,13 +1546,15 @@
     sel[i] = t;
     selcost[i] = K ? cost[p0 + t] : 1.0f;
 }
+constexpr uint32_t MOVED_FOREIGN = 8;
 void mrf_exact_costs(mvs_ctx* ctx, uint32_t nb0, uint32_t ne0) {
     resolve_best(ctx);
     if (ne0 <= nb0) return;
     if (ctx->exact_valid && ctx->exact_nb == nb0 && ctx->exact_ne == ne0) return;
     ctx->exact_valid = true; ctx->exact_nb = nb0; ctx->exact_ne = ne0;
-    MVS_HIP(hipMemsetAsync(ctx->m_moved.p + 6, 0, sizeof(uint32_t), ctx->stream));
-    hipLaunchKernelGGL(mrf_exact_cost_kernel, dim3((ne0 - nb0 + 255) / 256), dim3(256), 0, ctx->stream, ctx->r_ptr, ctx->r_view, ctx->r_cost, (const uint32_t*)ctx->b_lab, nb0, ne0, ctx->b_sel, ctx->b_cost, ctx->m_moved.p + 6);
+    ctx->m_moved.ensure(8 + 2 * 64);
+    MVS_HIP(hipMemsetAsync(ctx->m_moved.p + MOVED_FOREIGN, 0, sizeof(uint32_t), ctx->stream));
+    hipLaunchKernelGGL(mrf_exact_cost_kernel, dim3((ne0 - nb0 + 255) / 256), dim3(256), 0, ctx->stream, ctx->r_ptr, ctx->r_view, ctx->r_cost, (const uint32_t*)ctx->b_lab, nb0, ne0, ctx->b_sel, ctx->b_cost, ctx->m_moved.p + MOVED_FOREIGN);
     MVS_LAUNCH_CHECK();
 }
 
@@ -1501,7 +1639,7 @@
     resolve_best(ctx);
     MVS_HIP(hipMemsetAsync(bu, 0, 2 * sizeof(uint32_t), ctx->stream));
     if (ne0 > nb0) {
-        const uint32_t* foreign = (ctx->exact_valid && ctx->exact_nb == nb0 && ctx->exact_ne == ne0) ? ctx->m_moved.p + 6 : (const uint32_t*)nullptr;
+        const uint32_t* foreign = (ctx->exact_valid && ctx->exact_nb == nb0 && ctx->exact_ne == ne0) ? ctx->m_moved.p + MOVED_FOREIGN : (const uint32_t*)nullptr;
         hipLaunchKernelGGL(mrf_labels_kernel, dim3((ne0 - nb0 + 255) / 256), dim3(256), 0, ctx->stream, ctx->b_lab, nb0, ne0, ctx->csr_views, d_labels, bu, caller_order ? ctx->t_perm : (const uint32_t*)nullptr, foreign);
         MVS_LAUNCH_CHECK();
     }
diff --git a/mvs-texturing_amd/csrc/mgpu.hip b/mvs-texturing_amd/csrc/mgpu.hip
--- a/mvs-texturing_amd/csrc/mgpu.hip
+++ b/mvs-texturing_amd/csrc/mgpu.hip
@@ -14,6 +14,7 @@
 void mrf_icm_apply(mvs_ctx* ctx, uint32_t nb0, uint32_t ne0);
 void mrf_labels(mvs_ctx* ctx, uint32_t nb0, uint32_t ne0, uint32_t* d_labels, uint32_t out[2], bool caller_order = false);
 void resolve_best(mvs_ctx* ctx);
+uint64_t mrf_tables(mvs_ctx* ctx, int which, void* dst, uint64_t cap);
 void set_adjacency(mvs_ctx* ctx, const uint32_t* adj_ptr, const uint32_t* adj, int on_device, bool table_order);
 mvs_status api_fail(mvs_status st, const std::string& msg);
 
@@ -244,6 +245,13 @@
     MVS_API_END
 }
 
+mvs_status mvs_ctx_mrf_tables(mvs_ctx* ctx, int which, void* dst_host, uint64_t cap_bytes, uint64_t* bytes_out) {
+    if (!ctx || !bytes_out) return api_fail(MVS_ERR_INVALID, "null argument");
+    MVS_API_BEGIN
+    *bytes_out = mrf_tables(ctx, which, dst_host, cap_bytes);
+    MVS_API_END
+}
+
 mvs_status mvs_ctx_mrf_labels(mvs_ctx* ctx, uint32_t nb0, uint32_t ne0, uint32_t* labels, uint32_t* unseen_out) {
     if (!ctx || !labels || nb0 > ne0 || ne0 > ctx->csr_faces) return api_fail(MVS_ERR_INVALID, "bad argument");
     MVS_API_BEGIN
diff --git a/mvs-texturing_amd/viewsel.py b/mvs-texturing_amd/viewsel.py
--- a/mvs-texturing_amd/viewsel.py
+++ b/mvs-texturing_amd/viewsel.py
@@ -84,7 +84,7 @@
     "mvs_ctx_dc_get_max", "mvs_ctx_dc_set_max", "mvs_ctx_dc_get_histogram", "mvs_ctx_dc_set_histogram", "mvs_ctx_costs_export",
     "mvs_ctx_mrf_setup", "mvs_ctx_mrf_setup_marked", "mvs_ctx_mrf_sweep", "mvs_ctx_mrf_sweep_phase", "mvs_ctx_mrf_sweep_phase_part", "mvs_ctx_mrf_layout", "mvs_ctx_mrf_gather", "mvs_ctx_mrf_scatter",
     "mvs_ctx_mrf_energy", "mvs_ctx_mrf_keep_best", "mvs_ctx_mrf_step", "mvs_ctx_mrf_poll", "mvs_ctx_mrf_icm_gain", "mvs_ctx_mrf_icm_apply",
-    "mvs_ctx_mrf_labels"))
+    "mvs_ctx_mrf_labels", "mvs_ctx_mrf_tables"))
 
 
 _lib = None
@@ -138,6 +138,7 @@
         "mvs_ctx_mrf_step": [vp, vp], "mvs_ctx_mrf_poll": [vp, u32, C.POINTER(MrfProgress)],
         "mvs_ctx_mrf_icm_gain": [vp, u32, u32], "mvs_ctx_mrf_icm_apply": [vp, u32, u32, vp],
         "mvs_ctx_mrf_labels": [vp, u32, u32, vp, C.POINTER(u32)],
+        "mvs_ctx_mrf_tables": [vp, i32, vp, u64, C.POINTER(u64)],
         "mvs_ctx_prune_labels": [vp, u32], "mvs_undistort_image": [vp, C.c_int32, C.c_int32, C.c_float, C.c_float, C.c_float, vp],
         "mvs_postprocess_face_infos": [u32, u32, vp, vp, vp, vp, C.POINTER(Settings), C.POINTER(CCsr), C.POINTER(DcStats)],
         "mvs_comm_unique_id": [vp], "mvs_comm_create_rccl": [i32, i32, i32, vp, C.POINTER(vp)], "mvs_comm_create_local": [i32, C.POINTER(vp)], "mvs_comm_create_local_devices": [i32, vp, C.POINTER(vp)],
```

After: 76.51 million (median of 6 runs). No clear change (+0.6%).
